# wendongbi/Bridged-GNN

Hardware: AMD Instinct MI355X
Metric: aggregated_edges_per_sec_ktgnn_fwd (higher is better)
Workload: dtype f32; 1 GPU; C4 synthetic bridged graph (local) N=1000000 E'=20991058, 2-layer KT-GNN eval fwd F=128 hidden=128 C=2; parallelism=single, execution=eager launches

## Files before the change

### bridged_gnn_amd/_lib.py

```python
import ctypes as C
import os

import torch

_HERE = os.path.dirname(os.path.abspath(__file__))
SO_PATH = os.path.join(_HERE, "csrc", "libbgnn_hip.so")
_lib = None

_P, _I64, _I32, _F32, _SZ, _INT = C.c_void_p, C.c_int64, C.c_int32, C.c_float, C.c_size_t, C.c_int

SIGNATURES = {
    "bgnn_version": (_INT, []),
    "bgnn_source_hash": (C.c_char_p, []),
    "bgnn_error_string": (C.c_char_p, [_INT]),
    "bgnn_csr_workspace_bytes": (_SZ, [_I64, _I64]),
    "bgnn_build_dst_csr": (_INT, [_P, _I64, _I64, _INT, _P, _P, _P, _P, _P, _SZ, _P]),
    "bgnn_domain_sums_f64": (_INT, [_P, _I64, _I32, _I64, _P, _P, _P]),
    "bgnn_domain_sums_workspace_bytes": (_SZ, [_I32]),
    "bgnn_domain_sums_ws_f64": (_INT, [_P, _I64, _I32, _I64, _P, _P, _P, _SZ, _P]),
    "bgnn_domain_delta_f32": (_INT, [_P, _I32, _P, _P]),
    "bgnn_adaptedconv_transform_f32": (_INT, [_P, _I64, _I32, _I64, _P, _P, _P, _I32, _I32, _P, _P, _P, _P,
                                               _P, _P, _P, _P, _I64, _I64, _I64, _I64, _P, _P, _I32, _P, _P]),
    "bgnn_classifier_stage_f32": (_INT, [_P, _I64, _I32, _I64, _P, _P, _I32, _I32, _P, _P, _P, _P, _P, _P, _P, _P, _I64, _I64,
                                          _P, _P, _I32, _INT, _P, _P, _P, _P, _P, _P]),
    "bgnn_linear_narrow_transform_f32": (_INT, [_P, _I64, _I32, _I64, _P, _P, _I32, _INT, _P, _P, _P, _P, _P, _P]),
    "bgnn_narrow_transform_finish_f32": (_INT, [_P, _I64, _P, _P, _I32, _P, _P, _P, _P, _P, _P, _I64, _P, _P]),
    "bgnn_gram_workspace_bytes": (C.c_size_t, [_I32, _I32]),
    "bgnn_gram_f32": (_INT, [_P, _I64, _I32, _P, _I64, _I32, _I64, _P, _P, C.c_size_t, _P]),
    "bgnn_transform_bwd_prep_workspace_bytes": (C.c_size_t, [_I64, _I32]),
    "bgnn_transform_bwd_prep_f32": (_INT, [_P, _I64, _I64, _I32, _P, _P, _I64, _I32, _P, _P, _P, _P, _P, _P, _I32, _I64, _P, _I64, _P, _P, C.c_size_t, _P]),
    "bgnn_bn_acc_doubles": (_I64, [_I32]),
    "bgnn_bn_relu_dropout_f32": (_INT, [_P, _I64, _I32, _I64, _P, _P, _F32, _INT, _F32, C.c_uint64, _P, _F32, _P, _P, _P, _I64, _P, _P]),
    "bgnn_bn_relu_dropout_bwd_f32": (_INT, [_P, _P, _I64, _I32, _I64, _I64, _P, _P, _P, _F32, _INT, _F32, C.c_uint64, _P, _P, _I64, _P, _P]),
    "bgnn_bn_colstats_f32": (_INT, [_P, _I64, _I32, _I64, _P, _P]),
    "bgnn_bn_apply_rows_f32": (_INT, [_P, _I64, _I32, _I64, _P, _I64, _P, _P, _F32, _INT, _F32, C.c_uint64, _P, _P, _I64, _F32, _P, _P, _P, _I64, _P]),
    "bgnn_bn_bwd_reduce_rows_f32": (_INT, [_P, _P, _I64, _I32, _I64, _I64, _P, _I64, _P, _P, _F32, _INT, _F32, C.c_uint64, _P, _P, _I64, _P, _P]),
    "bgnn_bn_bwd_apply_rows_f32": (_INT, [_P, _P, _I64, _I32, _I64, _I64, _P, _P, _I64, _P, _P, _F32, _INT, _F32, C.c_uint64, _P, _P, _I64, _P, _I64, _P]),
    "bgnn_transform_bwd_consts_f32": (_INT, [_P, _P, _P, _P, _P, _I32, _I32, _P, _P, _P, _P]),
    "bgnn_transform_bwd_finish_f32": (_INT, [_P, _P, _P, _P, _P, _P, _P, _I32, _I32, _I32, _P, _P, _P, _P, _P, _P, _P, _I64, _P]),
    "bgnn_rowdot_f32": (_INT, [_P, _I64, _I64, _I32, _P, _I64, _I32, _P, _P]),
    "bgnn_linear_f32": (_INT, [_P, _I64, _I32, _I64, _P, _P, _I32, _INT, _P, _P, _P, _I64, _P]),
    "bgnn_adaptedconv_aggregate_f32": (_INT, [_P, _P, _I64, _P, _P, _P, _P, _P, _I64, _I64, _I32, _F32,
                                               _P, _I64, _P, _P, _P, _INT, _P, _INT, _I64, _I32, _P, _P, _P]),
    "bgnn_adaptedconv_aggregate_bounded_f32": (_INT, [_P, _P, _I64, _P, _P, _P, _P, _P, _I64, _I64, _I32, _F32,
                                                       _P, _I64, _P, _P, _P, _INT, _P, _INT, _I64, _I32, _P, _P, _I64, _I32, _P]),
    "bgnn_aggregate_tile_queue_words": (_I64, []),
    "bgnn_adaptedconv_aggregate_queued_f32": (_INT, [_P, _P, _I64, _P, _P, _P, _P, _P, _I64, _I64, _I32, _F32,
                                                      _P, _I64, _P, _P, _P, _INT, _P, _INT, _I64, _I32, _P, _P, _I64, _I64, _I32, _P]),
    "bgnn_aggregate_hub_workspace_bytes": (C.c_size_t, [_I64, _I32, _I64]),
    "bgnn_adaptedconv_aggregate_hub_f32": (_INT, [_P, _P, _I64, _P, _P, _P, _P, _P, _I64, _I32, _F32, _P, _I64, _P, _P, _INT, _P, _I32, _P,
                                                   _P, _I32, _P, _I64, _P, _P, _P, _I64, _P, _P, C.c_size_t, _P]),
    "bgnn_adaptedconv_aggregate_bwd_f32": (_INT, [_P, _P, _I64, _P, _P, _P, _P, _P, _I64, _I64, _I32, _F32,
                                                   _P, _I64, _P, _P, _I64, _P, _P, _P, _P, _P]),
    "bgnn_aggregate_bwd_pull_workspace_bytes": (C.c_size_t, [_I64, _I64, _I64, _I32, _I64, _I64]),
    "bgnn_adaptedconv_aggregate_bwd_pull_f32": (_INT, [_P, _P, _I64, _P, _P, _P, _P, _P, _P, _P, _P, _I64, _I64, _I32, _F32,
                                                        _P, _I64, _P, _P, _I64, _P, _P, _P, _P, _I32,
                                                        _P, _I64, _P, _P, _P, _I64, _P, _I64, _P, _P, _P, _I64, _P, C.c_size_t, _P]),
    "bgnn_aggregate_heads_bwd_workspace_bytes": (C.c_size_t, [_I64, _I64, _I32, _I64, _I64]),
    "bgnn_adaptedconv_aggregate_heads_bwd_f32": (_INT, [_P, _P, _P, _P, _P, _P, _P, _P, _P, _I64, _I64, _I32, _I32, _F32,
                                                         _P, _P, _P, _INT, _P, _P, _P, _P, _I32,
                                                         _P, _I64, _P, _P, _P, _I64, _P, _I64, _P, _P, _P, _I64, _P, C.c_size_t, _P]),
    "bgnn_adaptedconv_aggregate_heads_wide_f32": (_INT, [_P, _P, _I64, _P, _P, _P, _P, _P, _I64, _I32, _I32, _F32, _P, _P, _P]),
    "bgnn_aggregate_heads_wide_bwd_workspace_bytes": (C.c_size_t, [_I64, _I32, _I64]),
    "bgnn_adaptedconv_aggregate_heads_wide_bwd_f32": (_INT, [_P, _P, _I64, _P, _P, _P, _P, _P, _P, _P, _I64, _I32, _I32, _F32,
                                                              _P, _P, _P, _P, _P, _P, _P, _P, C.c_size_t, _P]),
    "bgnn_l2_normalize_rows_f32": (_INT, [_P, _I64, _I32, _F32, _P, _P]),
    "bgnn_topk_workspace_bytes": (_SZ, [_I64, _I64, _I32]),
    "bgnn_cosine_topk_f32": (_INT, [_P, _P, _I64, _I64, _I32, _I32, _INT, _P, _P, _P, _P, _SZ, _P]),
    "bgnn_mlp_pair_topk_f32": (_INT, [_P, _P, _P, _P, _P, _F32, _I64, _I64, _I32, _I32, _INT, _P, _P, _P,
                                       _P, _SZ, _P]),
    "bgnn_topk_edges_i64": (_INT, [_P, _I64, _I32, _I64, _I64, _P, _P]),
    "bgnn_topk_edges_coalesced_workspace_bytes": (_SZ, [_I64, _I32]),
    "bgnn_topk_edges_coalesced_i64": (_INT, [_P, _I64, _I32, _I64, _I64, _I64, _P, _P, _SZ, _P]),
    "bgnn_gather_rows_f32": (_INT, [_P, _I64, _I64, _P, _I64, _I32, _P, _I64, _P]),
    "bgnn_coalesce_workspace_bytes": (_SZ, [_I64]),
    "bgnn_coalesce_i64": (_INT, [_P, _I64, _I64, _P, _P, _SZ, _P]),
    "bgnn_sage_mean_aggregate_f32": (_INT, [_P, _I64, _I64, _P, _I64, _P, _P, _I64, _I32, _INT, _INT, _F32, C.c_uint64, _P,
                                             _P, _P, _I64, _P]),
    "bgnn_rows_segment_add_f32": (_INT, [_P, _I64, _I64, _P, _P, _P, _I64, _I32, _INT, _P, _I64, _I64, _P]),
    "bgnn_pair_mlp_workspace_bytes": (_SZ, [_I64]),
    "bgnn_pair_mlp_stats_f32": (_INT, [_P, _I64, _I64, _P, _I64, _I64, _P, _P, _I64, _F32, _P, _P, _P, _P, _SZ, _P]),
    "bgnn_pair_mlp_loss_f32": (_INT, [_P, _I64, _I64, _P, _I64, _I64, _P, _P, _P, _I64, _P, _P, _P, _P, _P, _F32, _P, _P, _P, _P,
                                       _SZ, _P]),
    "bgnn_pair_mlp_segsum_f32": (_INT, [_P, _I64, _I64, _P, _I64, _I64, _P, _P, _P, _I64, _P, _P, _P, _P, _P, _P, _F32, _P, _I64, _P]),
    "bgnn_pair_mlp_eval_f32": (_INT, [_P, _I64, _I64, _P, _I64, _I64, _P, _P, _P, _I64, _P, _P, _P, _P, _P, _P, _P, _SZ, _P]),
    "bgnn_pair_mlp_count_workspace_bytes": (_SZ, [_I64, _I64]),
    "bgnn_pair_mlp_count_f32": (_INT, [_P, _I64, _I64, _P, _I64, _I64, _P, _I64, _P, _I64, _P, _P, _P, _P, _P, _P, _P, _P, _SZ, _P]),
    "bgnn_pair_cos_loss_workspace_bytes": (_SZ, [_I64]),
    "bgnn_pair_cos_count_workspace_bytes": (_SZ, [_I64, _I64]),
    "bgnn_pair_cos_loss_f32": (_INT, [_P, _I64, _I64, _P, _I64, _I64, _P, _P, _P, _I64, _P, _P, _P, _P, _SZ, _P]),
    "bgnn_pair_cos_segsum_f32": (_INT, [_P, _I64, _I64, _P, _P, _P, _I64, _P, _I64, _P, _I64, _P]),
    "bgnn_pair_cos_count_f32": (_INT, [_P, _I64, _I64, _P, _I64, _I64, _P, _I64, _P, _I64, _P, _P, _P, _P, _SZ, _P]),
    "bgnn_sage_mean_aggregate_bwd_workspace_bytes": (_SZ, [_I64, _I32]),
    "bgnn_sage_mean_aggregate_bwd_f32": (_INT, [_P, _I64, _P, _I64, _P, _I64, _P, _P, _I64, _I32, _INT, _F32, _P, _I64, _P, _I64,
                                                 _P, _SZ, _P]),
    "bgnn_gcn_aggregate_workspace_bytes": (_SZ, [_I64, _I32]),
    "bgnn_gcn_aggregate_f32": (_INT, [_P, _I64, _I64, _P, _P, _P, _P, _I64, _I64, _I32, _INT, _F32, C.c_uint64, _P,
                                       _I32, _P, _I64, _P, _P, _I64, _P, _SZ, _P, _P, _I64, _P]),
    "bgnn_gcn_aggregate_bwd_f32": (_INT, [_P, _I64, _P, _I64, _I64, _P, _P, _P, _I64, _I64, _I32, _INT, _F32,
                                           _I32, _P, _I64, _P, _P, _I64, _P, _SZ, _P, _I64, _P, _I64, _P]),
    "bgnn_appnp_propagate_workspace_bytes": (_SZ, [_I64, _I32, _I64]),
    "bgnn_appnp_propagate_f32": (_INT, [_P, _I64, _P, _P, _P, _I64, _I64, _I32, _I32, _F32, _INT,
                                         _I32, _P, _I64, _P, _P, _I64, _P, _SZ, _P, _I64, _P]),
    "bgnn_appnp_log_softmax_bwd_f32": (_INT, [_P, _I64, _P, _I64, _I64, _I32, _P, _I64, _P]),
    "bgnn_feature_dropout_f32": (_INT, [_P, _P, _I64, _I32, _INT, _F32, C.c_uint64, _P, _P, _P]),
    "bgnn_feature_dropout_bwd_f32": (_INT, [_P, _P, _I64, _I32, _INT, _F32, C.c_uint64, _P, _P, _P]),
    "bgnn_appnp_step_f32": (_INT, [_P, _I64, _I64, _P, _I64, _P, _P, _P, _I64, _I64, _I32, _F32, _INT, _INT,
                                    _I32, _P, _I64, _P, _P, _I64, _P, _SZ, _P, _I64, _P]),
    "bgnn_feature_dropout_rows_f32": (_INT, [_P, _P, _P, _I64, _I32, _INT, _F32, C.c_uint64, _P, _P, _P]),
# ... 153 lines not shown
```

### bridged_gnn_amd/classifier_stage.py

```python
import os

import torch
import torch.nn.functional as F

from . import ops
from .ktgnn import _AggregateFn, _AggregateHeadsFn, _AggregateWideHeadsFn, _TransformPairFn, _pad_cols4, _plist


class ClassifierStage:

    def __init__(self, model):
        base = model.clf_base
        self.model, self.convs = model, (base, model.clf_target, model.clf_target)
        self.C, self.ld, self.slope = base.out_channels, ops.pad4(base.out_channels), base.negative_slope
        self.plain = not (base.root_weight or base.normalize)
        self.fused_log_softmax = ops.heads_log_softmax_supported(3, self.C)
        self.drop_caches()

    def drop_caches(self):
        self._a3_key = self._tf_key = self._tf_pack = None

    def views(self, t2s, s2t):
        ld = self.ld
        return [(t2s[:, j * ld:(j + 1) * ld], s2t[:, j * ld:(j + 1) * ld]) for j in range(3)]

    def attention(self, autograd=False):
        if autograd:
            return (torch.stack([c.a_f_t2s.weight.reshape(-1) for c in self.convs]),
                    torch.stack([c.a_f_s2t.weight.reshape(-1) for c in self.convs]))
        key = (self.convs[0]._versions(), self.convs[1]._versions())
        if self._a3_key != key:
            self._a3 = (torch.stack([c.a_f_t2s.weight.detach().reshape(-1) for c in self.convs]).contiguous(),
                        torch.stack([c.a_f_s2t.weight.detach().reshape(-1) for c in self.convs]).contiguous())
            self._a3_key = key
        return self._a3

    def finish(self, out3):
        logp = out3.view(out3.shape[0], 3, self.ld)[:, :, :self.C]
        if not self.fused_log_softmax:
            logp = F.log_softmax(logp, dim=2)
        return logp[:, 0], logp[:, 1], logp[:, 2]

    def fold_transformer(self):
        l0, bn, _, l3 = self.model.clf_transformer
        key = tuple((p.data_ptr(), p._version) for p in _plist(self.model.clf_transformer)) + \
            (bn.running_mean._version, bn.running_var._version)
        if self._tf_key != key:
            s = (bn.weight / torch.sqrt(bn.running_var + bn.eps)).detach()
            self._tf_w0 = (l0.weight.detach() * s[:, None]).float().contiguous()
            self._tf_w0t = self._tf_w0.t().contiguous()
            self._tf_b0 = (l0.bias.detach() * s + bn.bias.detach() - bn.running_mean * s).float().contiguous()
            self._tf_key = key
            self._tf_pack = None

    def transformer_hidden_eval(self, x, mask_u8=None, want_sums=False, sums_out=None):
        self.fold_transformer()
        sums = None
        dout, din = self._tf_w0.shape
        if x.dtype == torch.float32 and x.stride(1) == 1 and ops.linear_supported(din, dout):
            if want_sums:
                sums = sums_out if sums_out is not None else torch.zeros(2 * dout + 2, dtype=torch.float64, device=x.device)
            h1 = ops.linear(x, self._tf_w0, self._tf_b0, relu=True, mask_u8=mask_u8 if want_sums else None, colsum=sums)
        elif hasattr(torch, "_addmm_activation"):
            h1 = torch._addmm_activation(self._tf_b0, x, self._tf_w0t, use_gelu=False)
        else:
            h1 = F.relu(torch.addmm(self._tf_b0, x, self._tf_w0t))
        return (h1, sums) if want_sums else h1

    def transformer_eval(self, x):
        l3 = self.model.clf_transformer[3]
        return F.linear(self.transformer_hidden_eval(x), l3.weight, l3.bias)

    def composed_target_pack(self, din_pad):
        c, l3 = self.convs[1], self.model.clf_transformer[3]
        key = (din_pad, c._versions(), l3.weight._version, l3.bias._version, l3.weight.data_ptr())
        if self._tf_pack is None or self._tf_pack[0] != key:
            W3, b3 = l3.weight.detach(), l3.bias.detach()
            hd = c.head()
            din = W3.shape[0]

            def comp_gate(g):
                g = g.reshape(-1)
                return torch.cat((W3.t() @ g[:din], W3.t() @ g[din:])), (b3 * g[:din]).sum()
            g1, c1 = comp_gate(hd["g_s2t"])
            g2, c2 = comp_gate(hd["g_t2s"])
            head = {"W_s": hd["W_s"] @ W3, "W_t": hd["W_t"] @ W3,
                    "b_s": hd["W_s"] @ b3 + (hd["b_s"] if hd["b_s"] is not None else 0),
                    "b_t": hd["W_t"] @ b3 + (hd["b_t"] if hd["b_t"] is not None else 0),
                    "g_s2t": g1, "g_t2s": g2, "gate_const": (c1, c2)}
            self._tf_pack = (key, ops.pack_transform_heads([head], din_pad))
        return self._tf_pack[1]

    def one_pass(self, x, mask_u8, sums_h, views, arena):
        if sums_h is None or x.dtype != torch.float32 or x.stride(1) != 1:
            return None
        self.fold_transformer()
        dout, din = self._tf_w0.shape
        if x.shape[1] != din or dout != 128:
            return None
        pack_t = self.composed_target_pack(ops.pad4(dout))
        pair = self.convs[0].packed(x.shape[1], self.convs[1])
        if not ops.classifier_stage_supported(x, pair, self._tf_w0, pack_t):
            return None
        n_s = 2 * ops.pad4(dout) + 2
        sums_t = arena.take(n_s) if arena is not None else torch.zeros(n_s, dtype=torch.float64, device=x.device)
        raw = ops.classifier_stage(x, mask_u8, sums_h, pair, [views[0], views[1]], self._tf_w0, self._tf_b0, sums_t, pack_t, relu=True)
        return raw, None, sums_t

    def pair_tables(self, x, mask_u8, sums_h, views):
        self.convs[0].transform(x, mask_u8, sums=sums_h, partner=self.convs[1], out=[views[0], views[1]])

    def target_stage_a(self, x, mask_u8, sums_out=None):
        self.fold_transformer()
        dout, din = self._tf_w0.shape
        pack = self.composed_target_pack(ops.pad4(dout))
        if (sums_out is not None and x.dtype == torch.float32 and x.stride(1) == 1 and x.shape[1] == din
                and ops.linear_narrow_supported(din, dout, pack) and os.environ.get("BGNN_FUSED_TARGET", "1") != "0"):
            return ops.linear_narrow_transform(x, self._tf_w0, self._tf_b0, mask_u8, sums_out, pack, relu=True), None, sums_out
        h1, sums1 = self.transformer_hidden_eval(x, mask_u8, want_sums=True, sums_out=sums_out)
        h1 = _pad_cols4(h1)
        if sums1 is None or sums1.numel() != 2 * h1.shape[1] + 2:
            sums1 = ops.domain_sums(h1, mask_u8)
        return None, h1, sums1

    def target_stage_b(self, stage_a, mask_u8, out, sums_t=None):
        raw, h1, sums_t = (*stage_a[:2], sums_t if sums_t is not None else stage_a[2])
        if raw is not None:
            ops.narrow_transform_finish(raw, mask_u8, sums_t, self.composed_target_pack(ops.pad4(self._tf_w0.shape[0])), out)
        else:
            ops.adaptedconv_transform(h1, mask_u8, None, self.composed_target_pack(h1.shape[1]), out=[out], sums=sums_t)

    def target_tables(self, x, mask_u8, out, arena=None, sums_out=None):
        if sums_out is None:
            n_s = 2 * ops.pad4(self.model.clf_transformer[0].weight.shape[0]) + 2
            sums_out = arena.take(n_s) if arena is not None else torch.zeros(n_s, dtype=torch.float64, device=x.device)
        self.target_stage_b(self.target_stage_a(x, mask_u8, sums_out), mask_u8, out)

    def eval_tables(self, x, mask_u8, sums_h, views, arena):
        a = self.one_pass(x, mask_u8, sums_h, views, arena)
        if a is not None:
            return self.target_stage_b(a, mask_u8, views[2])
        self.pair_tables(x, mask_u8, sums_h, views)
        self.target_tables(x, mask_u8, views[2], arena)

    def train_walk(self, opt_in=False):
        if ops.heads_log_softmax_supported(3, self.C) and not (opt_in and os.environ.get("BGNN_FUSED_TRAIN_HEADS", "1") == "0"):
            return "narrow"
        if ops.wide_heads_supported(3, self.C) and not (opt_in and os.environ.get("BGNN_WIDE_TRAIN_HEADS", "0") != "1"):
            return "wide"
        return None if opt_in else "convs"

    def train_tables(self, x, mask_u8, sums_x, bn, sums_of=None, mean_hook=None):
        base, target, _ = self.convs
        l0, bnm, _, l3 = self.model.clf_transformer
        xt = l3(bn(l0(x), bnm, True, 0.0)).contiguous()
        sums_t = sums_of(xt) if sums_of is not None else None
        if mean_hook is None and _TransformPairFn.supported(x, base, target):
            prm = [t for c in (base, target)
                   for t in (c.lin_s.weight, c.lin_s.bias, c.lin_t.weight, c.lin_t.bias, c.a_g_s2t.weight, c.a_g_t2s.weight)]
            tabs_x = _TransformPairFn.apply(x, mask_u8, base, target, sums_x, *prm)
        else:
            tabs_x = (*base._transform_autograd(x, mask_u8, sums_x, mean_hook), *target._transform_autograd(x, mask_u8, sums_x, mean_hook))
        return (*tabs_x, *target._transform_autograd(xt, mask_u8, sums_t, mean_hook))

    def train_aggregate(self, walk, csr, mask_u8, tables, n_rows=None):
        C = self.C
        a_t, a_s = self.attention(autograd=True)
        if walk == "convs":
            return tuple(F.log_softmax(_AggregateFn.apply(tables[2 * j], tables[2 * j + 1], a_t[j], a_s[j], csr, mask_u8, C,
                                                          c.negative_slope)[:n_rows, :C], dim=1) for j, c in enumerate(self.convs))
        fn = _AggregateHeadsFn if walk == "narrow" else _AggregateWideHeadsFn
        logp = fn.apply(csr, mask_u8, C, self.slope, a_t, a_s, *tables)[:n_rows, :, :C]
        return logp[:, 0], logp[:, 1], logp[:, 2]
```

### bridged_gnn_amd/csrc/bgnn_aggregate.hip

```cpp
#include <cstdlib>
#include <cstring>
#include <type_traits>
#include "bgnn_common.h"

namespace {

struct AggParams {
  const float* h_t2s;
  const float* h_s2t;
  int64_t ldh;
  const float* a_t2s;
  const float* a_s2t;
  const int32_t* rowptr;
  const int32_t* col;
  const uint8_t* mask;
  int64_t row_begin;
  int64_t row_end;
  int32_t D;
  float slope;
  float* out;
  int64_t ldo;
  float* alpha;
  const float* ep_scale;
  const float* ep_shift;
// ... 1050 lines not shown
        __builtin_amdgcn_sched_barrier(0);
#pragma unroll
        for (int u = 0; u < U; ++u) asm volatile("buffer_load_dwordx4 %0, %1, %2, 0 offen" : "=v"(v[u]) : "v"(off[u]), "s"(rt) : "memory");
        xoff += (uint32_t)(STEP * 4);
        u32x4_t nq;
        request(nq);
        if constexpr (SLOW) asm volatile("s_waitcnt vmcnt(4)" : "+v"(v[0]), "+v"(v[1]), "+v"(v[2]), "+v"(v[3]) : : "memory");
        else asm volatile("s_waitcnt vmcnt(1)" : "+v"(v[0]), "+v"(v[1]), "+v"(v[2]), "+v"(v[3]) : : "memory");
        __builtin_amdgcn_sched_barrier(0);
        float l[U], cm = -INFINITY;
#pragma unroll
        for (int u = 0; u < U; ++u) {
          f2 z0 = f2{v[u].x, v[u].y} + h01, z1 = f2{v[u].z, v[u].w} + h23;
          z0 = __builtin_elementwise_max(z0, z0 * sl);
          z1 = __builtin_elementwise_max(z1, z1 * sl);
          float t = a4.x * z0.x;
          t = fmaf(a4.y, z0.y, t);
          t = fmaf(a4.z, z1.x, t);
          t = fmaf(a4.w, z1.y, t);
          l[u] = rem > u * EP ? t : -INFINITY;
          cm = fmaxf(cm, l[u]);
        }
        const float mn = fmaxf(m, cm);
        const float sc = (m == mn) ? 1.f : __expf(m - mn);
        const f2 sc2 = {sc, sc};
        acc01 *= sc2; acc23 *= sc2;
#pragma unroll
        for (int u = 0; u < U; ++u) {
          const float pe = (l[u] == -INFINITY) ? 0.f : __expf(l[u] - mn);
          s = u == 0 ? fmaf(s, sc, pe) : s + pe;
          acc01.x = fmaf(pe, v[u].x, acc01.x); acc01.y = fmaf(pe, v[u].y, acc01.y);
          acc23.x = fmaf(pe, v[u].z, acc23.x); acc23.y = fmaf(pe, v[u].w, acc23.y);
        }
        m = mn;
        rem -= STEP;
        uint32_t nid[U];
        take(nq, nid);
        offsets(nid);
      }
    };
    if (any) {
      if (slow) walk(std::true_type{});
      else walk(std::false_type{});
    }
    float4 acc = make_float4(acc01.x, acc01.y, acc23.x, acc23.y);
#pragma unroll
    for (int o = 1; o < EP; o <<= 1) {
      const int src = (sub ^ o) * HEADS + h + g * GL;
      const int from = lane_on ? src : lane;
      const float m2 = __shfl(m, from), s2 = __shfl(s, from);
      float4 b;
      b.x = __shfl(acc.x, from); b.y = __shfl(acc.y, from); b.z = __shfl(acc.z, from); b.w = __shfl(acc.w, from);
      const float mn = fmaxf(m, m2);
      const float c1 = (m == mn) ? 1.f : __expf(m - mn), c2 = (m2 == mn) ? 1.f : __expf(m2 - mn);
      s = fmaf(s, c1, s2 * c2);
      acc.x = fmaf(acc.x, c1, b.x * c2); acc.y = fmaf(acc.y, c1, b.y * c2);
      acc.z = fmaf(acc.z, c1, b.z * c2); acc.w = fmaf(acc.w, c1, b.w * c2);
      m = mn;
    }
    if (rvalid && sub == 0) {
#pragma clang fp contract(off)
      const float inv = 1.f / (s + 1e-16f);
      float4 r4 =make_float4(acc.x * inv, acc.y * inv, acc.z * inv, acc.w * inv);
      if (p.ep_relu == 2) {
        float mx = r4.x;
        if (p.D > 1) mx = fmaxf(mx, r4.y);
        if (p.D > 2) mx = fmaxf(mx, r4.z);
        if (p.D > 3) mx = fmaxf(mx, r4.w);
        float se = expf(r4.x - mx);
        if (p.D > 1) se += expf(r4.y - mx);
        if (p.D > 2) se += expf(r4.z - mx);
        if (p.D > 3) se += expf(r4.w - mx);
        const float lse = logf(se);
        r4.x = r4.x - mx - lse;
        r4.y = p.D > 1 ? r4.y - mx - lse : 0.f;
        r4.z = p.D > 2 ? r4.z - mx - lse : 0.f;
        r4.w = p.D > 3 ? r4.w - mx - lse : 0.f;
      }
      __builtin_amdgcn_raw_buffer_store_b128(__builtin_bit_cast(u32x4_t, r4), ro, ((uint32_t)i * (uint32_t)HEADS + (uint32_t)h) * 16u, 0, 0);
    }
  }
}

inline int tq_chunk_for(int64_t ntiles, int64_t grid) {
  static const int forced = [] { const char* e = getenv("BGNN_AGG_CHUNK"); return e ? atoi(e) : 0; }();
  (void)ntiles; (void)grid;
  return forced > 0 ? forced : 4;
}

template <int HEADS, int EP, int U>
int launch_heads(const AggParams& p, hipStream_t st) {
  constexpr int RPB = 4 * (64 / (EP * HEADS));
  static const int cap = [] {
    int per_cu = 0, dev = 0;
    hipDeviceProp_t prop;
    if (hipGetDevice(&dev) != hipSuccess || hipGetDeviceProperties(&prop, dev) != hipSuccess) return 2048;
    if (hipOccupancyMaxActiveBlocksPerMultiprocessor(&per_cu, agg_heads_lanes_kernel<HEADS, EP, U>, 256, 0) != hipSuccess || per_cu < 1) return 2048;
    if (per_cu > 8) per_cu = 8;
    return per_cu * prop.multiProcessorCount / 8 * 8;
  }();
  const int64_t ntiles = (p.row_end - p.row_begin + p.n_vrows + RPB - 1) / RPB;
  int64_t grid = ntiles < cap ? (ntiles + 7) / 8 * 8 : cap;
  if (grid < 8) grid = 8;
  hipLaunchKernelGGL((agg_heads_lanes_kernel<HEADS, EP, U>), dim3((unsigned)grid), dim3(256), 0, st, p);
  BGNN_LAUNCH_CHECK();
  return 0;
}

template <int LF, int EP, int U>
int resident_blocks() {
  static const int nb = [] {
    int per_cu = 0, dev = 0;
    hipDeviceProp_t prop;
    if (hipGetDevice(&dev) != hipSuccess || hipGetDeviceProperties(&prop, dev) != hipSuccess) return 2048;
    if (hipOccupancyMaxActiveBlocksPerMultiprocessor(&per_cu, agg_kernel<LF, EP, U>, 256, 0) != hipSuccess || per_cu < 1)
      return 2048;
    if (per_cu > 8) per_cu = 8;
    return per_cu * prop.multiProcessorCount / 8 * 8;
  }();
  return nb;
}

template <int LF, int EP, int U>
int launch(const AggParams& p, hipStream_t st) {
  constexpr int RPB = 4 * (64 / (LF * EP));
  int64_t ntiles = ((p.row_end - p.row_begin) * p.heads + RPB - 1) / RPB;
  const int64_t cap = resident_blocks<LF, EP, U>();
  int64_t grid = ntiles < cap ? (ntiles + 7) / 8 * 8 : cap;
  if (grid < 8) grid = 8;
  AggParams q = p;
  q.tq_chunk = tq_chunk_for(ntiles, grid);
  hipLaunchKernelGGL((agg_kernel<LF, EP, U>), dim3((unsigned)grid), dim3(256), 0, st, q);
  BGNN_LAUNCH_CHECK();
  return 0;
}

template <int LF, int U>
int launch_wide(const AggParams& p, hipStream_t st) {
  constexpr int RPB = 4 * (64 / LF);
  static const int cap = [] {
    int per_cu = 0, dev = 0;
    hipDeviceProp_t prop;
    if (hipGetDevice(&dev) != hipSuccess || hipGetDeviceProperties(&prop, dev) != hipSuccess) return 2048;
    if (hipOccupancyMaxActiveBlocksPerMultiprocessor(&per_cu, agg_wide_kernel<LF, U>, 256, 0) != hipSuccess || per_cu < 1) return 2048;
    if (per_cu > 8) per_cu = 8;
    const char* e = getenv("BGNN_AGG_BLOCKS_PER_CU");
    if (e && atoi(e) > 0 && atoi(e) < per_cu) per_cu = atoi(e);
    return per_cu * prop.multiProcessorCount / 8 * 8;
  }();
  const int64_t ntiles = ((p.row_end - p.row_begin) * p.heads + p.n_vrows + RPB - 1) / RPB;
  int64_t grid = ntiles < cap ? (ntiles + 7) / 8 * 8 : cap;
  if (grid < 8) grid = 8;
  AggParams q = p;
  q.tq_chunk = tq_chunk_for(ntiles, grid);
  static const int il = [] { const char* e = getenv("BGNN_AGG_INTERLEAVE"); return e ? atoi(e) : 1; }();
  q.tq_interleave = il;
  static const int nseg = [] { const char* e = getenv("BGNN_XCD_SEGMENTS"); return e ? atoi(e) : 8; }();
  q.xcd_segments = nseg;
  hipLaunchKernelGGL((agg_wide_kernel<LF, U>), dim3((unsigned)grid), dim3(256), 0, st, q);
  BGNN_LAUNCH_CHECK();
  return 0;
}

static bool fast_plan(AggParams& p, int64_t table_rows) {
  static const bool on = [] { const char* e = getenv("BGNN_AGG_FAST"); return !(e && atoi(e) == 0); }();
  if (!on || table_rows <= 0) return false;
  if (p.heads != 1 || p.mode != 0 || p.n_vrows != 0 || p.hub_threshold != 0) return false;
  const int64_t lim24 = (int64_t)1 << 24, lim32 = ((int64_t)1 << 32) - 1;
  if (table_rows > lim24 || p.row_end > table_rows || p.ldh * 4 >= lim24 || p.ldo * 4 >= lim24) return false;
  const char* a = reinterpret_cast<const char*>(p.h_t2s);
  const char* b = reinterpret_cast<const char*>(p.h_s2t);
  const char* lo = a < b ? a : b;
  const int64_t span = (int64_t)((a < b ? b : a) - lo) + table_rows * p.ldh * 4;
  if (span > lim32 || p.row_end * p.ldo * 4 > lim32) return false;
  p.tbl_base = lo;
  p.tbl_bytes = (uint32_t)span;
  p.off_t2s = (uint32_t)(a - lo);
  p.off_s2t = (uint32_t)(b - lo);
  const int64_t lane_max = (span - table_rows * p.ldh * 4) + p.ldh * 4, dead = (((int64_t)1 << 32) - 16) - lane_max;
  p.dead_off = dead >= span ? (uint32_t)dead : 0u;
  return true;
}

static bool heads_fast_plan(AggParams& p, int64_t table_rows) {
  static const bool on = [] { const char* e = getenv("BGNN_HEADS_FAST"); return !(e && atoi(e) == 0); }();
  if (!on || table_rows <= 0) return false;
  if ((p.heads != 2 && p.heads != 3) || p.D > 4 || p.ldh != 4 || p.ldo != 4) return false;
  if (p.mode != 0 || p.n_vrows != 0 || p.hub_threshold != 0 || p.alpha != nullptr) return false;
  if (!(p.slope >= 0.f && p.slope <= 1.f)) return false;
  const int64_t lim24 = (int64_t)1 << 24, lim32 = ((int64_t)1 << 32) - 1;
  const int64_t rs = (int64_t)p.heads * 16;
  if (table_rows > lim24 || p.row_end > table_rows) return false;
  const char* a = reinterpret_cast<const char*>(p.h_t2s);
  const char* b = reinterpret_cast<const char*>(p.h_s2t);
  const char* lo = a < b ? a : b;
  const int64_t span = (int64_t)((a < b ? b : a) - lo) + table_rows * rs;
  if (span > lim32 || p.row_end * rs > lim32) return false;
  p.tbl_base = lo;
  p.tbl_bytes = (uint32_t)span;
  p.off_t2s = (uint32_t)(a - lo);
  p.off_s2t = (uint32_t)(b - lo);
  p.dead_off = (uint32_t)span;
  return true;
}

constexpr int kClaimTileDefault = 1;
struct ClaimCfg { int tile, nq, ahead; };
static const ClaimCfg& claim_cfg() {
  static const ClaimCfg c = [] {
    ClaimCfg r{kClaimTileDefault, 4, 1};
    if (const char* e = getenv("BGNN_AGG_CLAIM")) r.tile = strcmp(e, "chunk") == 0 ? 0 : (strcmp(e, "tile") == 0 ? 1 : r.tile);
    if (const char* e = getenv("BGNN_AGG_SUBQUEUES")) { const int v = atoi(e); if (v >= 1 && v <= 8) r.nq = v; }
    if (const char* e = getenv("BGNN_AGG_CLAIM_AHEAD")) r.ahead = atoi(e) != 0;
    return r;
  }();
  return c;
}
static int64_t claim_queue_words() { return (int64_t)8 * claim_cfg().nq * TQ_SPACING_WORDS; }

template <int LF, bool ALPHA>
int launch_wide_fast(const AggParams& p, hipStream_t st) {
  constexpr int RPB = 4 * (64 / LF);
  static const int per_cu_max = [] {
    int per_cu = 0;
    if (hipOccupancyMaxActiveBlocksPerMultiprocessor(&per_cu, agg_wide_fast_kernel<LF, ALPHA>, 256, 0) != hipSuccess || per_cu < 1) return 0;
    if (per_cu > 8) per_cu = 8;
    const char* e = getenv("BGNN_AGG_BLOCKS_PER_CU");
    if (e && atoi(e) > 0 && atoi(e) < per_cu) per_cu = atoi(e);
    return per_cu;
  }();
  static const int n_cu = [] {
    int dev = 0;
    hipDeviceProp_t prop;
    if (hipGetDevice(&dev) != hipSuccess || hipGetDeviceProperties(&prop, dev) != hipSuccess) return 0;
    return prop.multiProcessorCount;
  }();
  static const bool forced = getenv("BGNN_AGG_BLOCKS_PER_CU") != nullptr;
  int per_cu = per_cu_max;
  if (p.gather_hint == 2 && !forced && per_cu > 3) per_cu = 3;
  const int64_t cap = (per_cu_max > 0 && n_cu > 0) ? (int64_t)per_cu * n_cu / 8 * 8 : 2048;
  const int64_t ntiles = (p.row_end - p.row_begin + RPB - 1) / RPB;
  int64_t grid = ntiles < cap ? (ntiles + 7) / 8 * 8 : cap;
  if (grid < 8) grid = 8;
  AggParams q = p;
  q.tq_chunk = tq_chunk_for(ntiles, grid);
  static const int il = [] { const char* e = getenv("BGNN_AGG_INTERLEAVE"); return e ? atoi(e) : 1; }();
  q.tq_interleave = il;
  static const int nseg = [] { const char* e = getenv("BGNN_XCD_SEGMENTS"); return e ? atoi(e) : 8; }();
  q.xcd_segments = nseg;
  const ClaimCfg& cc = claim_cfg();
  const bool tile_claims = cc.tile && p.tile_queue != nullptr && p.tq_words >= claim_queue_words();
  q.tq_subqueues = tile_claims ? cc.nq : 0;
  q.tq_ahead = cc.ahead;
  hipLaunchKernelGGL((agg_wide_fast_kernel<LF, ALPHA>), dim3((unsigned)grid), dim3(256), 0, st, q);
  BGNN_LAUNCH_CHECK();
  return 0;
}

struct HubMergeParams {
  const int32_t* hub_rows; const int32_t* seg_ptr; int64_t n_hubs;
  const float* part_acc;
  const float* part_ms;
  const uint8_t* mask;
  int32_t D; int64_t ldo; int32_t heads;
  float* out; const float* ep_scale; const float* ep_shift; int ep_relu;
  double* colsum; float* state_ms;
  float* alpha; const int32_t* rowptr;
};

template <int LF>
__global__ __launch_bounds__(256) void hub_merge_wide_kernel(HubMergeParams p) {
  const int lane = threadIdx.x % LF, grp = threadIdx.x / LF;
  constexpr int GPB = 256 / LF;
  const int f0 = lane * 4;
// ... 52 lines not shown
      *reinterpret_cast<float4*>(p.out + node * p.ldo + f0) = o;
      if (p.mask[node] != 0) { cs_s.x += o.x; cs_s.y += o.y; cs_s.z += o.z; cs_s.w += o.w; n_s += 1.f; }
      else                   { cs_t.x += o.x; cs_t.y += o.y; cs_t.z += o.z; cs_t.w += o.w; n_t += 1.f; }
    }
  }
  if (p.colsum != nullptr) {
    unsafeAtomicAdd(&red[0][f0], cs_s.x); unsafeAtomicAdd(&red[0][f0 + 1], cs_s.y);
    unsafeAtomicAdd(&red[0][f0 + 2], cs_s.z); unsafeAtomicAdd(&red[0][f0 + 3], cs_s.w);
    unsafeAtomicAdd(&red[1][f0], cs_t.x); unsafeAtomicAdd(&red[1][f0 + 1], cs_t.y);
    unsafeAtomicAdd(&red[1][f0 + 2], cs_t.z); unsafeAtomicAdd(&red[1][f0 + 3], cs_t.w);
    if (lane == 0) { unsafeAtomicAdd(&red[0][LF * 4], n_s); unsafeAtomicAdd(&red[1][LF * 4], n_t); }
    __syncthreads();
    for (int t = threadIdx.x; t < 2 * (LF * 4 + 1); t += 256) {
      const int d = t / (LF * 4 + 1), c = t % (LF * 4 + 1);
      const double sum = (double)red[d][c];
      if (c == LF * 4) unsafeAtomicAdd(&p.colsum[2 * p.ldo + d], sum);
      else if (c < p.ldo) unsafeAtomicAdd(&p.colsum[d * p.ldo + c], sum);
    }
  }
}

__global__ __launch_bounds__(256) void hub_merge_heads_kernel(HubMergeParams p) {
  const int64_t t = (int64_t)blockIdx.x * 256 + threadIdx.x;
  if (t >= p.n_hubs * p.heads) return;
  const int64_t hrow = t / p.heads;
  const int h = (int)(t - hrow * p.heads);
  const int64_t node = p.hub_rows[hrow];
  float m = -INFINITY, s = 0.f;
  float4 acc = make_float4(0.f, 0.f, 0.f, 0.f);
  for (int32_t v = p.seg_ptr[hrow]; v < p.seg_ptr[hrow + 1]; ++v) {
    const int64_t e = (int64_t)v * p.heads + h;
    const float m2 = p.part_ms[2 * e], s2 = p.part_ms[2 * e + 1];
    const float4 b = *reinterpret_cast<const float4*>(p.part_acc + e * p.ldo);
    const float mn = fmaxf(m, m2);
    const float c1 = (m == mn) ? 1.f : __expf(m - mn), c2 = (m2 == mn) ? 1.f : __expf(m2 - mn);
    s = s * c1 + s2 * c2;
    acc.x = acc.x * c1 + b.x * c2; acc.y = acc.y * c1 + b.y * c2;
    acc.z = acc.z * c1 + b.z * c2; acc.w = acc.w * c1 + b.w * c2;
    m = mn;
  }
  const float inv = 1.f / (s + 1e-16f);
  float4 r = make_float4(acc.x * inv, acc.y * inv, acc.z * inv, acc.w * inv);
  if (p.state_ms != nullptr) {
    p.state_ms[2 * (node * p.heads + h)] = m;
    p.state_ms[2 * (node * p.heads + h) + 1] = s;
  }
  if (p.ep_relu == 2) {
    float mx = r.x;
    if (p.D > 1) mx = fmaxf(mx, r.y);
    if (p.D > 2) mx = fmaxf(mx, r.z);
    if (p.D > 3) mx = fmaxf(mx, r.w);
    float se = expf(r.x - mx);
    if (p.D > 1) se += expf(r.y - mx);
    if (p.D > 2) se += expf(r.z - mx);
    if (p.D > 3) se += expf(r.w - mx);
    const float lse = logf(se);
    r.x = r.x - mx - lse;
    r.y = p.D > 1 ? r.y - mx - lse : 0.f;
    r.z = p.D > 2 ? r.z - mx - lse : 0.f;
    r.w = p.D > 3 ? r.w - mx - lse : 0.f;
  }
  *reinterpret_cast<float4*>(p.out + (node * p.heads + h) * p.ldo) = r;
}

template <int HEADS, int EP, int U>
int launch_heads_fast(const AggParams& p, hipStream_t st) {
  constexpr int RPB = 4 * (64 / (EP * HEADS));
  static const int cap = [] {
    int per_cu = 0, dev = 0;
    hipDeviceProp_t prop;
    if (hipGetDevice(&dev) != hipSuccess || hipGetDeviceProperties(&prop, dev) != hipSuccess) return 2048;
    if (hipOccupancyMaxActiveBlocksPerMultiprocessor(&per_cu, agg_heads_fast_kernel<HEADS, EP, U>, 256, 0) != hipSuccess || per_cu < 1) return 2048;
    if (per_cu > 8) per_cu = 8;
    return per_cu * prop.multiProcessorCount / 8 * 8;
  }();
  const int64_t ntiles = (p.row_end - p.row_begin + RPB - 1) / RPB;
  int64_t grid = ntiles < cap ? (ntiles + 7) / 8 * 8 : cap;
  if (grid < 8) grid = 8;
  hipLaunchKernelGGL((agg_heads_fast_kernel<HEADS, EP, U>), dim3((unsigned)grid), dim3(256), 0, st, p);
  BGNN_LAUNCH_CHECK();
  return 0;
}

static int dispatch_aggregate(const AggParams& p, hipStream_t st, int64_t table_rows = 0) {
  const int32_t D = p.D, heads = p.heads;
  if ((heads == 3 || heads == 2) && D <= 4 && p.ldh == 4 && p.ldo == 4) {
    AggParams q = p;
    if (heads_fast_plan(q, table_rows)) return heads == 3 ? launch_heads_fast<3, 2, 4>(q, st) : launch_heads_fast<2, 2, 4>(q, st);
    return heads == 3 ? launch_heads<3, 2, 4>(p, st) : launch_heads<2, 2, 4>(p, st);
  }
  const int nv = (D + 3) / 4;
  if (nv <= 1) return launch<1, 4, 4>(p, st);
  if (nv <= 2) return launch<2, 2, 4>(p, st);
  if (nv <= 4) return launch<4, 1, 8>(p, st);
  if (nv <= 8) return launch<8, 1, 4>(p, st);
  const bool wide_ok = p.slope >= 0.f && p.slope <= 1.f && (int64_t)heads * p.ldh * 4 < (int64_t)1 << 32;
  if (wide_ok) {
    AggParams q = p;
    if (fast_plan(q, table_rows)) {
      if (q.alpha != nullptr) {
        if (nv <= 16) return launch_wide_fast<16, true>(q, st);
        if (nv <= 32) return launch_wide_fast<32, true>(q, st);
        return launch_wide_fast<64, true>(q, st);
      }
      if (nv <= 16) return launch_wide_fast<16, false>(q, st);
      if (nv <= 32) return launch_wide_fast<32, false>(q, st);
      return launch_wide_fast<64, false>(q, st);
    }
    if (nv <= 16) return launch_wide<16, 4>(p, st);
    if (nv <= 32) return launch_wide<32, 4>(p, st);
    return launch_wide<64, 4>(p, st);
  }
  if (nv <= 16) return launch<16, 1, 8>(p, st);
  if (nv <= 32) return launch<32, 1, 4>(p, st);
  return launch<64, 1, 4>(p, st);
}

static bool hub_capable(int32_t D, int64_t ldh, int64_t ldo, int32_t heads, float slope) {
  if ((heads == 3 || heads == 2) && D <= 4 && ldh == 4 && ldo == 4) return true;
  const int nv = (D + 3) / 4;
  return heads == 1 && nv > 8 && slope >= 0.f && slope <= 1.f && ldh * 4 < (int64_t)1 << 32;
}

}

static int aggregate_impl(const float* h_t2s, const float* h_s2t, int64_t ldh,
                          const float* a_t2s, const float* a_s2t,
                          const int32_t* rowptr, const int32_t* col, const uint8_t* mask,
                          int64_t row_begin, int64_t row_end, int32_t D, float negative_slope,
                          float* out, int64_t ldo, float* alpha_opt,
                          const float* ep_scale_opt, const float* ep_shift_opt, int ep_relu,
                          float* state_ms_opt, int part, int64_t park_begin, int32_t heads,
                          double* colsum_opt, uint32_t* tile_queue_opt, int64_t tile_queue_words, int64_t table_rows, int32_t gather_hint,
                          void* stream) {
  if (colsum_opt && heads != 1) return BGNN_E_SHAPE;
  if (tile_queue_opt && tile_queue_words < 8) return BGNN_E_WORKSPACE;
  if (part == 1 && (park_begin < row_begin || park_begin > row_end)) return BGNN_E_SHAPE;
  if (part < 0 || part > 3 || (part != 0 && (!state_ms_opt || alpha_opt))) return BGNN_E_NULL;
  if (part == 3 && !((heads == 3 || heads == 2) && D <= 4 && ldh == 4 && ldo == 4)) return BGNN_E_SHAPE;
  if (heads < 1 || heads > 8 || (heads > 1 && (alpha_opt || ep_scale_opt))) return BGNN_E_SHAPE;
  if (ep_relu < 0 || ep_relu > 2) return BGNN_E_SHAPE;
  if (ep_relu == 2 && !((heads == 3 || heads == 2) && D <= 4 && ldh == 4 && ldo == 4)) return BGNN_E_SHAPE;
  if (!h_t2s || !h_s2t || !a_t2s || !a_s2t || !rowptr || !col || !mask || !out) return BGNN_E_NULL;
  if (row_begin < 0 || row_end < row_begin || D <= 0 || D > 256 || ldh < D || ldo < D) return BGNN_E_SHAPE;
  if ((ldh & 3) || (ldo & 3) || !bgnn_aligned16(h_t2s) || !bgnn_aligned16(h_s2t) || !bgnn_aligned16(out))
    return BGNN_E_ALIGN;
  if ((ep_scale_opt == nullptr) != (ep_shift_opt == nullptr)) return BGNN_E_NULL;
  if (row_end == row_begin) return 0;
  AggParams p{h_t2s, h_s2t, ldh, a_t2s, a_s2t, rowptr, col, mask, row_begin, row_end, D, negative_slope,
              out, ldo, alpha_opt, ep_scale_opt, ep_shift_opt, ep_relu, tile_queue_opt, colsum_opt, heads, state_ms_opt, part,
              park_begin, 4};
  p.gather_hint = gather_hint;
  p.tq_words = tile_queue_words;
  hipStream_t st = (hipStream_t)stream;
  if (tile_queue_opt) {
    const int64_t zw = claim_cfg().tile && tile_queue_words >= claim_queue_words() ? claim_queue_words() : 8;
    hipError_t e = bgnn_zero_async(tile_queue_opt, (size_t)zw * sizeof(uint32_t), st);
    if (e != hipSuccess) return (int)e;
  }
  return dispatch_aggregate(p, st, table_rows);
}

extern "C" int bgnn_adaptedconv_aggregate_f32(const float* h_t2s, const float* h_s2t, int64_t ldh,
                                              const float* a_t2s, const float* a_s2t,
                                              const int32_t* rowptr, const int32_t* col, const uint8_t* mask,
                                              int64_t row_begin, int64_t row_end, int32_t D, float negative_slope,
                                              float* out, int64_t ldo, float* alpha_opt,
                                              const float* ep_scale_opt, const float* ep_shift_opt, int ep_relu,
                                              float* state_ms_opt, int part, int64_t park_begin, int32_t heads,
                                              double* colsum_opt, uint32_t* tile_queue_opt, void* stream) {
  return aggregate_impl(h_t2s, h_s2t, ldh, a_t2s, a_s2t, rowptr, col, mask, row_begin, row_end, D, negative_slope, out, ldo, alpha_opt,
                        ep_scale_opt, ep_shift_opt, ep_relu, state_ms_opt, part, park_begin, heads, colsum_opt, tile_queue_opt, 8, 0, 0, stream);
}

extern "C" int bgnn_adaptedconv_aggregate_bounded_f32(const float* h_t2s, const float* h_s2t, int64_t ldh,
                                                      const float* a_t2s, const float* a_s2t,
                                                      const int32_t* rowptr, const int32_t* col, const uint8_t* mask,
                                                      int64_t row_begin, int64_t row_end, int32_t D, float negative_slope,
                                                      float* out, int64_t ldo, float* alpha_opt,
                                                      const float* ep_scale_opt, const float* ep_shift_opt, int ep_relu,
                                                      float* state_ms_opt, int part, int64_t park_begin, int32_t heads,
                                                      double* colsum_opt, uint32_t* tile_queue_opt, int64_t table_rows, int32_t gather_hint,
                                                      void* stream) {
  if (table_rows < row_end || gather_hint < 0 || gather_hint > 2) return BGNN_E_SHAPE;
  return aggregate_impl(h_t2s, h_s2t, ldh, a_t2s, a_s2t, rowptr, col, mask, row_begin, row_end, D, negative_slope, out, ldo, alpha_opt,
                        ep_scale_opt, ep_shift_opt, ep_relu, state_ms_opt, part, park_begin, heads, colsum_opt, tile_queue_opt, 8, table_rows, gather_hint, stream);
}

extern "C" int64_t bgnn_aggregate_tile_queue_words(void) { return claim_cfg().tile ? claim_queue_words() : 8; }

extern "C" int bgnn_adaptedconv_aggregate_queued_f32(const float* h_t2s, const float* h_s2t, int64_t ldh,
                                                     const float* a_t2s, const float* a_s2t,
                                                     const int32_t* rowptr, const int32_t* col, const uint8_t* mask,
                                                     int64_t row_begin, int64_t row_end, int32_t D, float negative_slope,
                                                     float* out, int64_t ldo, float* alpha_opt,
                                                     const float* ep_scale_opt, const float* ep_shift_opt, int ep_relu,
                                                     float* state_ms_opt, int part, int64_t park_begin, int32_t heads,
                                                     double* colsum_opt, uint32_t* tile_queue_opt, int64_t tile_queue_words,
                                                     int64_t table_rows, int32_t gather_hint, void* stream) {
  if (table_rows < row_end || gather_hint < 0 || gather_hint > 2) return BGNN_E_SHAPE;
  return aggregate_impl(h_t2s, h_s2t, ldh, a_t2s, a_s2t, rowptr, col, mask, row_begin, row_end, D, negative_slope, out, ldo, alpha_opt,
                        ep_scale_opt, ep_shift_opt, ep_relu, state_ms_opt, part, park_begin, heads, colsum_opt, tile_queue_opt,
                        tile_queue_words, table_rows, gather_hint, stream);
}

extern "C" size_t bgnn_aggregate_hub_workspace_bytes(int64_t n_segments, int32_t heads, int64_t ldo) {
  const size_t nv = (size_t)(n_segments > 0 ? n_segments : 0), h = (size_t)(heads > 0 ? heads : 1);
  return bgnn_align_up(sizeof(float) * nv * h * (size_t)(ldo > 0 ? ldo : 0), 256) + bgnn_align_up(sizeof(float) * 2 * nv * h, 256) + 256;
}

extern "C" int bgnn_adaptedconv_aggregate_hub_f32(const float* h_t2s, const float* h_s2t, int64_t ldh,
                                                  const float* a_t2s, const float* a_s2t,
                                                  const int32_t* rowptr, const int32_t* col, const uint8_t* mask,
                                                  int64_t N, int32_t D, float negative_slope, float* out, int64_t ldo,
                                                  const float* ep_scale_opt, const float* ep_shift_opt, int ep_relu,
                                                  float* state_ms_opt, int32_t heads, double* colsum_opt,
                                                  uint32_t* tile_queue_opt, int32_t hub_threshold, const int32_t* hub_rows,
                                                  int64_t n_hubs, const int32_t* hub_seg_ptr, const int32_t* seg_bounds,
                                                  const int32_t* seg_node, int64_t n_segments, float* alpha_opt,
                                                  void* ws, size_t ws_bytes, void* stream) {
  if (!h_t2s || !h_s2t || !a_t2s || !a_s2t || !rowptr || !col || !mask || !out) return BGNN_E_NULL;
  if (alpha_opt && heads != 1) return BGNN_E_SHAPE;
  if (n_hubs > 0 && (!hub_rows || !hub_seg_ptr || !seg_bounds || !seg_node || !ws)) return BGNN_E_NULL;
  if (N < 0 || D <= 0 || D > 256 || ldh < D || ldo < D || (ldh & 3) || (ldo & 3) || hub_threshold < 2 || n_hubs < 0 || n_segments < n_hubs)
    return BGNN_E_SHAPE;
  if (!hub_capable(D, ldh, ldo, heads, negative_slope)) return BGNN_E_SHAPE;
  if (colsum_opt && heads != 1) return BGNN_E_SHAPE;
  if (heads > 1 && ep_scale_opt) return BGNN_E_SHAPE;
  if (ep_relu < 0 || ep_relu > 2 || (ep_relu == 2 && heads == 1)) return BGNN_E_SHAPE;
  if ((ep_scale_opt == nullptr) != (ep_shift_opt == nullptr)) return BGNN_E_NULL;
  if (!bgnn_aligned16(h_t2s) || !bgnn_aligned16(h_s2t) || !bgnn_aligned16(out) || (ws && !bgnn_aligned16(ws))) return BGNN_E_ALIGN;
  if (n_hubs > 0 && ws_bytes < bgnn_aggregate_hub_workspace_bytes(n_segments, heads, ldo)) return BGNN_E_WORKSPACE;
  if (N == 0) return 0;
  hipStream_t st = (hipStream_t)stream;
  const int part = (state_ms_opt && heads > 1) ? 3 : 0;
  AggParams p{h_t2s, h_s2t, ldh, a_t2s, a_s2t, rowptr, col, mask, 0, N, D, negative_slope,
              out, ldo, alpha_opt, ep_scale_opt, ep_shift_opt, ep_relu, tile_queue_opt, colsum_opt, heads, state_ms_opt, part,
              0, 4};
  p.hub_threshold = n_hubs > 0 ? hub_threshold : 0;
  if (tile_queue_opt) {
    hipError_t e = bgnn_zero_async(tile_queue_opt, 8 * sizeof(uint32_t), st);
    if (e != hipSuccess) return (int)e;
  }
  float* part_acc = n_hubs > 0 ? (float*)ws : nullptr;
  float* part_ms = n_hubs > 0 ? (float*)((char*)ws + bgnn_align_up(sizeof(float) * (size_t)n_segments * (size_t)heads * (size_t)ldo, 256)) : nullptr;
  if (n_hubs > 0) {
    p.vrow_node = seg_node; p.vrow_bounds = seg_bounds; p.n_vrows = n_segments; p.vout = part_acc; p.vms = part_ms;
  }
  int rc = dispatch_aggregate(p, st, N);
  if (rc || n_hubs == 0) return rc;
  HubMergeParams mp{hub_rows, hub_seg_ptr, n_hubs, part_acc, part_ms, mask, D, ldo, heads, out, ep_scale_opt, ep_shift_opt,
                    ep_relu, colsum_opt, part == 3 ? state_ms_opt : nullptr, alpha_opt, rowptr};
  if (heads > 1) {
    hipLaunchKernelGGL(hub_merge_heads_kernel, dim3((unsigned)((n_hubs * heads + 255) / 256)), dim3(256), 0, st, mp);
  } else {
    const int nvs = (D + 3) / 4;
    int64_t grid = n_hubs < 2048 ? n_hubs : 2048;
    if (nvs <= 16) hipLaunchKernelGGL(hub_merge_wide_kernel<16>, dim3((unsigned)((grid + 15) / 16)), dim3(256), 0, st, mp);
    else if (nvs <= 32) hipLaunchKernelGGL(hub_merge_wide_kernel<32>, dim3((unsigned)((grid + 7) / 8)), dim3(256), 0, st, mp);
    else hipLaunchKernelGGL(hub_merge_wide_kernel<64>, dim3((unsigned)((grid + 3) / 4)), dim3(256), 0, st, mp);
  }
  BGNN_LAUNCH_CHECK();
  return 0;
}

#ifdef BGNN_TUNING
extern "C" int bgnn_tune_reset_counters(void* stream) { (void)stream; return 0; }
extern "C" int bgnn_tune_aggregate(const float* h_t2s, const float* h_s2t, int64_t ldh, const float* a_t2s,
                                   const float* a_s2t, const int32_t* rowptr, const int32_t* col, const uint8_t* mask,
// ... 41 lines not shown
```

### bridged_gnn_amd/csrc/bgnn_transform.hip

```cpp
#include <cstdlib>
#include <type_traits>
#include "bgnn_common.h"
#include "bgnn_transform_params.h"

using bgnn_tf::GemmParams;
using bgnn_tf::MAXH;
using bgnn_tf::f32x16;
using bgnn_tf::tanh_fast;

namespace {

constexpr int DS_NT = 1024;
__global__ __launch_bounds__(DS_NT) void domain_sums_kernel(const float* __restrict__ x, int64_t N, int32_t Din,
                                                          int64_t ldx, const uint8_t* __restrict__ mask,
                                                          double* __restrict__ sums, double* __restrict__ part) {
  if (part != nullptr) sums = part + (int64_t)blockIdx.x * (2 * Din + 2);
  const int nc4 = Din >> 2;
  const int cw = nc4 < 256 ? nc4 : 256;
  const int rl = DS_NT / cw;
  const int tid = threadIdx.x;
  const int cl = tid % cw, r0 = tid / cw;
  const bool active = r0 < rl;
  const int64_t rows_per_block = (N + gridDim.x - 1) / gridDim.x;
  const int64_t rb = blockIdx.x * rows_per_block;
// ... 834 lines not shown
                                              const uint8_t* mask, const float* delta_opt, const double* sums_opt,
                                              int32_t n_heads, int32_t D, const float* Wp, const float* bias_p,
                                              const float* gates, const float* gate_const_opt,
                                              float* h_s2t_0, float* h_t2s_0, float* h_s2t_1, float* h_t2s_1,
                                              int64_t ldh, int64_t row_stride, int64_t n_tail_t2s, int64_t n_tail_s2t,
                                              const int32_t* tile_need_opt, const int64_t* team_runs_host_opt, int32_t n_team_runs,
                                              float* small_ws, void* stream) {
  if ((delta_opt != nullptr) == (sums_opt != nullptr)) return BGNN_E_NULL;
  if (delta_opt && !bgnn_aligned16(delta_opt)) return BGNN_E_ALIGN;
  if (n_team_runs < 0 || n_team_runs > 2 || (n_team_runs > 0 && !team_runs_host_opt)) return BGNN_E_SHAPE;
  if (tile_need_opt && (n_tail_t2s || n_tail_s2t)) return BGNN_E_SHAPE;
  if (n_tail_t2s < 0 || n_tail_s2t < 0 || n_tail_t2s + n_tail_s2t > N) return BGNN_E_SHAPE;
  if (!x || !mask || !Wp || !bias_p || !gates || !h_s2t_0 || !h_t2s_0 || !small_ws) return BGNN_E_NULL;
  if (n_heads < 1 || n_heads > MAXH || (n_heads == 2 && (!h_s2t_1 || !h_t2s_1))) return BGNN_E_NULL;
  if (N < 0 || Din <= 0 || D <= 0 || ldx < Din || ldh < D) return BGNN_E_SHAPE;
  if ((Din & 3) || (ldx & 3) || (ldh & 3) || (row_stride & 3) || row_stride < ldh) return BGNN_E_SHAPE;
  if (!bgnn_aligned16(x) || !bgnn_aligned16(Wp) || !bgnn_aligned16(gates)) return BGNN_E_ALIGN;
  if (N == 0) return 0;
  hipStream_t st = (hipStream_t)stream;
  const int NC = n_heads * 2 * (int)ldh;
  float* wd = small_ws;
  float* gc = small_ws + NC;
  hipLaunchKernelGGL(wd_kernel, dim3((unsigned)((NC + 2 * n_heads + 3) / 4)), dim3(256), 0, st, Wp, NC, Din, delta_opt, sums_opt, gates,
                     gate_const_opt, n_heads, wd, gc);
  BGNN_LAUNCH_CHECK();
  GemmParams p{};
  p.x = x; p.ldx = ldx; p.N = N; p.Din = Din; p.mask = mask; p.Wp = Wp; p.bias = bias_p; p.wd = wd; p.g = gates; p.gc = gc;
  p.out[0][0] = h_s2t_0; p.out[0][1] = h_t2s_0; p.out[1][0] = h_s2t_1; p.out[1][1] = h_t2s_1;
  p.ldh = ldh; p.row_stride = row_stride; p.NC = NC; p.n_heads = n_heads; p.relu = 0; p.colsum = nullptr; p.col_off = 0;
  const int64_t nrt = (N + BM - 1) / BM;
  const int64_t nrt8 = (nrt + 7) / 8 * 8;
  const bool wreg = NC % 64 == 0 && Din <= 128;
  p.tail_t2s_begin = 0; p.tail_s2t_begin = 0;
  if ((n_tail_t2s || n_tail_s2t) && n_heads == 1 && wreg) {
    p.tail_t2s_begin = N - n_tail_t2s - n_tail_s2t;
    p.tail_s2t_begin = N - n_tail_s2t;
    if (p.tail_s2t_begin == 0) p.tail_s2t_begin = 1, p.tail_t2s_begin = p.tail_t2s_begin > 1 ? 1 : p.tail_t2s_begin;
  }
  static const bool use_stream = [] { const char* e = getenv("BGNN_GEMM_STREAM"); return !e || atoi(e) != 0; }();
  p.tile_need = tile_need_opt;
  for (int r = 0; r < n_team_runs; ++r) {
    p.team_begin[r] = team_runs_host_opt[3 * r]; p.team_end[r] = team_runs_host_opt[3 * r + 1]; p.team_table[r] = (int32_t)team_runs_host_opt[3 * r + 2];
  }
  if (use_stream && bgnn_tf_stream_supported(p)) return bgnn_tf_stream_launch(p, st, n_cu());
  if (wreg) return launch_wreg<0>(p, st);
  if (NC <= 24 && Din <= 128) {
    const int64_t nt = (N + 31) / 32, nb = (nt + 3) / 4;
    const unsigned grid = (unsigned)(nb < 2 * n_cu() ? nb : 2 * n_cu());
    if (Din <= 64) hipLaunchKernelGGL((transform_skinny_kernel<64>), dim3(grid), dim3(256), 0, st, p);
    else hipLaunchKernelGGL((transform_skinny_kernel<128>), dim3(grid), dim3(256), 0, st, p);
  } else if (NC <= 32) {
    hipLaunchKernelGGL((transform_gemm_kernel<32, 4, 1, 1, 1>), dim3((unsigned)nrt8), dim3(256), 0, st, p);
  } else if (NC <= 64) {
    hipLaunchKernelGGL((transform_gemm_kernel<64, 2, 2, 2, 1>), dim3((unsigned)nrt8), dim3(256), 0, st, p);
  } else {
    const int nct = (NC + 127) / 128;
    hipLaunchKernelGGL((transform_gemm_kernel<128, 2, 2, 2, 2>), dim3((unsigned)(nrt8 * nct)), dim3(256), 0, st, p);
  }
  BGNN_LAUNCH_CHECK();
  return 0;
}

extern "C" int bgnn_linear_f32(const float* x, int64_t N, int32_t Din, int64_t ldx, const float* W, const float* bias,
                               int32_t Dout, int relu, const uint8_t* mask_opt, double* colsum_opt,
                               float* out, int64_t ldo, void* stream) {
  if (!x || !W || !bias || !out || (colsum_opt && !mask_opt)) return BGNN_E_NULL;
  if (N < 0 || Din <= 0 || Din > 128 || (Din & 3) || (ldx & 3) || ldx < Din || Dout <= 0 || (Dout & 63) || ldo < Dout || (ldo & 3))
    return BGNN_E_SHAPE;
  if (!bgnn_aligned16(x) || !bgnn_aligned16(W) || !bgnn_aligned16(bias) || !bgnn_aligned16(out)) return BGNN_E_ALIGN;
  if (N == 0) return 0;
  GemmParams p{};
  p.x = x; p.ldx = ldx; p.N = N; p.Din = Din; p.mask = mask_opt; p.Wp = W; p.bias = bias; p.wd = nullptr; p.g = nullptr; p.gc = nullptr;
  p.out[0][0] = out; p.out[0][1] = out; p.out[1][0] = out; p.out[1][1] = out;
  p.ldh = Dout;
  p.row_stride = ldo; p.NC = Dout; p.n_heads = 1; p.relu = relu; p.colsum = colsum_opt;
  return launch_wreg<1>(p, (hipStream_t)stream);
}

namespace {
__global__ __launch_bounds__(256) void narrow_finish_kernel(const float* __restrict__ raw, int64_t N,
                                                            const uint8_t* __restrict__ mask,
                                                            const float* __restrict__ bias, const float* __restrict__ wd,
                                                            const float* __restrict__ gc, float* __restrict__ out_s2t,
                                                            float* __restrict__ out_t2s, int64_t row_stride) {
  const float4 b0 = *reinterpret_cast<const float4*>(bias), b1 = *reinterpret_cast<const float4*>(bias + 4);
  const float4 w0 = *reinterpret_cast<const float4*>(wd), w1 = *reinterpret_cast<const float4*>(wd + 4);
  const float g0 = gc[0], g1 = gc[1];
  for (int64_t r = blockIdx.x * (int64_t)blockDim.x + threadIdx.x; r < N; r += (int64_t)gridDim.x * blockDim.x) {
    const float4 a = *reinterpret_cast<const float4*>(raw + r * 12);
    const float4 b = *reinterpret_cast<const float4*>(raw + r * 12 + 4);
    const float2 pg = *reinterpret_cast<const float2*>(raw + r * 12 + 8);
    const bool sdom = mask[r] != 0;
    const float c0 = sdom ? -tanh_fast(pg.x + g0) : 0.f;
    const float c1 = sdom ? 0.f : tanh_fast(pg.y + g1);
    float4 o0, o1;
    o0.x = fmaf(c0, w0.x, a.x + b0.x); o0.y = fmaf(c0, w0.y, a.y + b0.y);
    o0.z = fmaf(c0, w0.z, a.z + b0.z); o0.w = fmaf(c0, w0.w, a.w + b0.w);
    o1.x = fmaf(c1, w1.x, b.x + b1.x); o1.y = fmaf(c1, w1.y, b.y + b1.y);
    o1.z = fmaf(c1, w1.z, b.z + b1.z); o1.w = fmaf(c1, w1.w, b.w + b1.w);
    *reinterpret_cast<float4*>(out_s2t + r * row_stride) = o0;
    *reinterpret_cast<float4*>(out_t2s + r * row_stride) = o1;
  }
}
}

extern "C" int bgnn_linear_narrow_transform_f32(const float* x, int64_t N, int32_t Din, int64_t ldx, const float* W,
                                                const float* bias, int32_t Dout, int relu, const uint8_t* mask,
                                                double* colsum, const float* Wp2, const float* gates2,
                                                float* raw, void* stream) {
  if (!x || !W || !bias || !mask || !colsum || !Wp2 || !gates2 || !raw) return BGNN_E_NULL;
  if (N < 0 || Din <= 0 || Din > 128 || (Din & 3) || (ldx & 3) || ldx < Din || (Dout != 64 && Dout != 128 && Dout != 256))
    return BGNN_E_SHAPE;
  if (!bgnn_aligned16(x) || !bgnn_aligned16(W) || !bgnn_aligned16(bias) || !bgnn_aligned16(raw)) return BGNN_E_ALIGN;
  if (N == 0) return 0;
  GemmParams p{};
  p.x = x; p.ldx = ldx; p.N = N; p.Din = Din; p.mask = mask; p.Wp = W; p.bias = bias;
  p.ldh = Dout; p.row_stride = Dout; p.NC = Dout; p.n_heads = 1; p.relu = relu ? 1 : 0; p.colsum = colsum;
  p.w2 = Wp2; p.g2 = gates2; p.raw = raw;
  return launch_wreg<2>(p, (hipStream_t)stream);
}

extern "C" int bgnn_classifier_stage_f32(const float* x, int64_t N, int32_t Din, int64_t ldx, const uint8_t* mask,
                                         const double* sums_x, int32_t sk_heads, int32_t sk_D, const float* sk_Wp,
                                         const float* sk_bias, const float* sk_gates, const float* sk_gate_const_opt,
                                         float* h_s2t_0, float* h_t2s_0, float* h_s2t_1, float* h_t2s_1, int64_t sk_ldh,
                                         int64_t sk_row_stride, const float* W, const float* bias, int32_t Dout, int relu,
                                         double* colsum, const float* Wp2, const float* gates2, float* raw, float* small_ws,
                                         void* stream) {
  if (!x || !mask || !sums_x || !sk_Wp || !sk_bias || !sk_gates || !h_s2t_0 || !h_t2s_0 || !W || !bias || !colsum || !Wp2 || !gates2 ||
      !raw || !small_ws) return BGNN_E_NULL;
  if (sk_heads < 1 || sk_heads > MAXH || (sk_heads == 2 && (!h_s2t_1 || !h_t2s_1))) return BGNN_E_NULL;
  if (N < 0 || Din <= 0 || (Din & 3) || (ldx & 3) || ldx < Din || sk_D <= 0 || sk_ldh < sk_D || (sk_ldh & 3) || (sk_row_stride & 3) ||
      sk_row_stride < sk_ldh) return BGNN_E_SHAPE;
  if (!bgnn_aligned16(x) || !bgnn_aligned16(sk_Wp) || !bgnn_aligned16(sk_bias) || !bgnn_aligned16(raw) || !bgnn_aligned16(small_ws))
    return BGNN_E_ALIGN;
  if (N == 0) return 0;
  hipStream_t st = (hipStream_t)stream;
  const int sk_NC = sk_heads * 2 * (int)sk_ldh;
  float* wd = small_ws;
  float* gc = small_ws + sk_NC;
  GemmParams p{};
  p.x = x; p.ldx = ldx; p.N = N; p.Din = Din; p.mask = mask; p.Wp = W; p.bias = bias;
  p.ldh = Dout; p.row_stride = Dout; p.NC = Dout; p.n_heads = 1; p.relu = relu ? 1 : 0; p.colsum = colsum;
  p.w2 = Wp2; p.g2 = gates2; p.raw = raw;
  p.sk_Wp = sk_Wp; p.sk_bias = sk_bias; p.sk_wd = wd; p.sk_g = sk_gates; p.sk_gc = gc;
  p.sk_out[0][0] = h_s2t_0; p.sk_out[0][1] = h_t2s_0; p.sk_out[1][0] = h_s2t_1; p.sk_out[1][1] = h_t2s_1;
  p.sk_ldh = sk_ldh; p.sk_row_stride = sk_row_stride; p.sk_NC = sk_NC; p.sk_heads = sk_heads;
  if (!bgnn_tf_cls_supported(p)) return BGNN_E_SHAPE;
  hipLaunchKernelGGL(wd_kernel, dim3((unsigned)((sk_NC + 2 * sk_heads + 3) / 4)), dim3(256), 0, st, sk_Wp, sk_NC, Din, (const float*)nullptr,
                     sums_x, sk_gates, sk_gate_const_opt, sk_heads, wd, gc);
  BGNN_LAUNCH_CHECK();
  return bgnn_tf_cls_launch(p, st, n_cu());
}

extern "C" int bgnn_narrow_transform_finish_f32(const float* raw, int64_t N, const uint8_t* mask, const double* sums,
                                                int32_t Din, const float* Wp2, const float* bias2, const float* gates2,
                                                const float* gate_const_opt, float* h_s2t, float* h_t2s,
                                                int64_t row_stride, float* small_ws, void* stream) {
  if (!raw || !mask || !sums || !Wp2 || !bias2 || !gates2 || !h_s2t || !h_t2s || !small_ws) return BGNN_E_NULL;
  if (N < 0 || Din <= 0 || (Din & 3) || row_stride < 4 || (row_stride & 3)) return BGNN_E_SHAPE;
  if (!bgnn_aligned16(raw) || !bgnn_aligned16(h_s2t) || !bgnn_aligned16(h_t2s) || !bgnn_aligned16(bias2) ||
      !bgnn_aligned16(small_ws)) return BGNN_E_ALIGN;
  if (N == 0) return 0;
  hipStream_t st = (hipStream_t)stream;
  float* wd = small_ws;
  float* gc = small_ws + 8;
  hipLaunchKernelGGL(wd_kernel, dim3(3), dim3(256), 0, st, Wp2, 8, Din, (const float*)nullptr, sums, gates2, gate_const_opt, 1, wd, gc);
  BGNN_LAUNCH_CHECK();
  const int64_t nb = (N + 255) / 256;
  hipLaunchKernelGGL(narrow_finish_kernel, dim3((unsigned)(nb < 4096 ? nb : 4096)), dim3(256), 0, st, raw, N, mask, bias2, wd, gc,
                     h_s2t, h_t2s, row_stride);
  BGNN_LAUNCH_CHECK();
  return 0;
}
```

### bridged_gnn_amd/csrc/bgnn_transform_cls.hip

```cpp
#include <cstdio>
#include <cstdlib>
#include "bgnn_common.h"
#include "bgnn_transform_params.h"

using bgnn_tf::GemmParams;
using bgnn_tf::MAXH;
using bgnn_tf::f32x16;
using bgnn_tf::tanh_fast;

namespace {

typedef _Float16 h8 __attribute__((ext_vector_type(8)));
typedef _Float16 h4 __attribute__((ext_vector_type(4)));

constexpr int CLS_TARGET_EXP = 10;
constexpr int DK = 128, KB16 = DK / 16, NCT = 4;
constexpr int PIECE = 32 * DK * 2;
constexpr int SLOT = 32 * 36 * 4 + 2 * 32 * 4;
constexpr int T_LD = 36;

__device__ __forceinline__ int chunk_off(int r, int c) { return r * 256 + ((c ^ (r & 15)) << 4); }
__device__ __forceinline__ void pow2_scales(float mx, float& sc, float& inv) {
  int E = (__builtin_bit_cast(int, mx) >> 23) & 0xff;
  E = E < 40 ? 40 : E;
// ... 159 lines not shown
  float cs_s[NCT], cs_t[NCT], cnt_s = 0.f, cnt_t = 0.f;
#pragma unroll
  for (int ct = 0; ct < NCT; ++ct) cs_s[ct] = cs_t[ct] = 0.f;

  if (tile < ntiles) gload(tile);
  for (; tile < ntiles; tile += stride) {
    CLS_MARK(0);
    const bool sdom = rmk != 0;
    const int64_t row = tile * 32 + fr;
    const bool valid = row < p.N;
    float mx = 0.f;
#pragma unroll
    for (int kb = 0; kb < KB16; ++kb)
#pragma unroll
      for (int c = 0; c < 2; ++c) {
        if (!din_full && 16 * kb + 8 * fh + 4 * c >= p.Din) ra[kb][c] = make_float4(0.f, 0.f, 0.f, 0.f);
        mx = fmaxf(fmaxf(fabsf(ra[kb][c].x), fabsf(ra[kb][c].y)), mx);
        mx = fmaxf(fmaxf(fabsf(ra[kb][c].z), fabsf(ra[kb][c].w)), mx);
      }
    mx = fmaxf(mx, __shfl_xor(mx, 32));
    float scx, s_row;
    pow2_scales(mx, scx, s_row);
    h8 xh[KB16], xl[KB16];
#pragma unroll
    for (int kb = 0; kb < KB16; ++kb)
#pragma unroll
      for (int c = 0; c < 2; ++c) {
        const float f[4] = {ra[kb][c].x, ra[kb][c].y, ra[kb][c].z, ra[kb][c].w};
#pragma unroll
        for (int e = 0; e < 4; ++e) {
          const _Float16 h = (_Float16)(f[e] * scx);
          xh[kb][4 * c + e] = h;
          xl[kb][4 * c + e] = (_Float16)fmaf(f[e], scx, -(float)h);
        }
      }
    if (fh == 0) {
      cfs[fr] = (valid && sdom) ? 1.f : 0.f;
      cfs[32 + fr] = (valid && !sdom) ? 1.f : 0.f;
      cnt_s += (valid && sdom) ? 1.f : 0.f;
      cnt_t += (valid && !sdom) ? 1.f : 0.f;
    }
    const int64_t tnext = tile + stride < ntiles ? tile + stride : tile;
    if constexpr (!PAIR) gload(tnext);
    __builtin_amdgcn_fence(__ATOMIC_RELEASE, "workgroup", "local");
    constexpr int HK = KB16 / 2;
    h8 wf[2][HK][2];
    auto fetch_w = [&](int hc, int buf) {
      const int op = hc >> 1, half = hc & 1;
      const unsigned char* wb = wl + ((op == 0 ? NCT : op - 1) * 2) * PIECE;
#pragma unroll
      for (int j = 0; j < HK; ++j) {
        wf[buf][j][0] = *reinterpret_cast<const h8*>(wb + roff(HK * half + j));
        wf[buf][j][1] = *reinterpret_cast<const h8*>(wb + PIECE + roff(HK * half + j));
      }
    };
    auto half_chain = [&](int hc, f32x16& acc, auto&& between) {
      if constexpr (PAIR) {
        __builtin_amdgcn_sched_barrier(0);
        fetch_w(hc, 0);
      } else if (hc + 1 < 2 * (NCT + 1)) fetch_w(hc + 1, (hc + 1) & 1);
      __builtin_amdgcn_sched_barrier(0);
      const int half = hc & 1, buf = PAIR ? 0 : hc & 1;
#pragma unroll
      for (int j = 0; j < HK; ++j) {
        const int kb = HK * half + j;
        acc = __builtin_amdgcn_mfma_f32_32x32x16_f16(wf[buf][j][0], xl[kb], acc, 0, 0, 0);
        acc = __builtin_amdgcn_mfma_f32_32x32x16_f16(wf[buf][j][1], xh[kb], acc, 0, 0, 0);
        acc = __builtin_amdgcn_mfma_f32_32x32x16_f16(wf[buf][j][0], xh[kb], acc, 0, 0, 0);
        between(kb);
      }
    };
    auto nothing = [](int) {};
    CLS_MARK(1);
    if constexpr (!PAIR) fetch_w(0, 0);
    {
      f32x16 acc;
#pragma unroll
      for (int r = 0; r < 16; ++r) acc[r] = 0.f;
      half_chain(0, acc, nothing);
      half_chain(1, acc, nothing);
      CLS_MARK(2);
      const float ss = s_row * cinvS;
      if (valid) {
        float cf = 0.f;
#pragma unroll
        for (int q = 0; q < 3; ++q) {
          if (optr[q] != nullptr) {
            if (newq[q]) {
              const float pre = hsel[q] == 0 ? acc[12] : hsel[q] == 1 ? acc[13] : hsel[q] == 2 ? acc[14] : acc[15];
              cf = (sdom != t1q[q]) ? tanh_fast(fmaf(pre, ss, gcq[q])) : 0.f;
              cf = t1q[q] ? cf : -cf;
            }
            const float4 bq = *reinterpret_cast<const float4*>(&skc[0][8 * q + 4 * fh]), wq = *reinterpret_cast<const float4*>(&skc[1][8 * q + 4 * fh]);
            float4 o;
            o.x = fmaf(cf, wq.x, fmaf(acc[4 * q], ss, bq.x));     o.y = fmaf(cf, wq.y, fmaf(acc[4 * q + 1], ss, bq.y));
            o.z = fmaf(cf, wq.z, fmaf(acc[4 * q + 2], ss, bq.z)); o.w = fmaf(cf, wq.w, fmaf(acc[4 * q + 3], ss, bq.w));
            *reinterpret_cast<float4*>(optr[q] + row * p.sk_row_stride) = o;
          }
        }
      }
    }
    float o2[8];
#pragma unroll
    for (int i = 0; i < 8; ++i) o2[i] = 0.f;
    const float sc1 = s_row * cinvW;
    struct Stage2 { float a1[16]; float mx, sc2, inv2; h8 ah[2], al[2]; f32x16 acc2; h8 w2h[2], w2l[2]; };
    auto stage2_step = [&](Stage2& q, int ct, int j) {
      if (j == 0) {
        q.mx = fmaxf(q.mx, __shfl_xor(q.mx, 32));
#pragma unroll
        for (int kb = 0; kb < 2; ++kb) { q.w2h[kb] = w2lds[ct][kb][0][lane]; q.w2l[kb] = w2lds[ct][kb][1][lane]; }
      } else if (j == 1) {
        pow2_scales(q.mx, q.sc2, q.inv2);
#pragma unroll
        for (int r = 0; r < 16; ++r) q.acc2[r] = 0.f;
      } else if (j == 2 || j == 3) {
        const int kb = j - 2;
#pragma unroll
        for (int e = 0; e < 8; ++e) {
          const _Float16 h = (_Float16)(q.a1[8 * kb + e] * q.sc2);
          q.ah[kb][e] = h;
          q.al[kb][e] = (_Float16)fmaf(q.a1[8 * kb + e], q.sc2, -(float)h);
        }
      } else if (j == 4 || j == 5) {
        const int kb = j - 4;
        q.acc2 = __builtin_amdgcn_mfma_f32_32x32x16_f16(q.w2h[kb], q.al[kb], q.acc2, 0, 0, 0);
        q.acc2 = __builtin_amdgcn_mfma_f32_32x32x16_f16(q.w2l[kb], q.ah[kb], q.acc2, 0, 0, 0);
        q.acc2 = __builtin_amdgcn_mfma_f32_32x32x16_f16(q.w2h[kb], q.ah[kb], q.acc2, 0, 0, 0);
      } else if (j == 6) {
#pragma unroll
        for (int r = 0; r < 16; ++r) {
          const float v = tsc[(16 * fh + r) * T_LD + fr];
          cs_s[ct] = fmaf(cfs[16 * fh + r], v, cs_s[ct]);
          cs_t[ct] = fmaf(cfs[32 + 16 * fh + r], v, cs_t[ct]);
        }
        if constexpr (PAIR) asm volatile("" : "+v"(cs_s[ct]), "+v"(cs_t[ct]));
      } else {
        const float s2 = q.inv2 * cinv2;
#pragma unroll
        for (int i = 0; i < 8; ++i) o2[i] = fmaf(q.acc2[i], s2, o2[i]);
        if constexpr (PAIR) asm volatile("" : "+v"(o2[0]), "+v"(o2[1]), "+v"(o2[2]), "+v"(o2[3]), "+v"(o2[4]), "+v"(o2[5]), "+v"(o2[6]), "+v"(o2[7]));
      }
    };
    Stage2 q2;
    f32x16 acc;
#pragma unroll
    for (int r = 0; r < 16; ++r) acc[r] = 0.f;
    CLS_MARK(3);
    half_chain(2, acc, nothing);
    half_chain(3, acc, nothing);
    CLS_MARK(4);
#pragma unroll
    for (int ct = 0; ct < NCT; ++ct) {
      __builtin_amdgcn_fence(__ATOMIC_RELEASE, "workgroup", "local");
      q2.mx = 0.f;
#pragma unroll
      for (int qq = 0; qq < 4; ++qq) {
        const float4 b4 = *reinterpret_cast<const float4*>(&bias1[32 * ct + 8 * qq + 4 * fh]);
        const float bb[4] = {b4.x, b4.y, b4.z, b4.w};
#pragma unroll
        for (int e = 0; e < 4; ++e) {
          float v = fmaf(acc[4 * qq + e], sc1, bb[e]);
          if (relu) v = fmaxf(v, 0.f);
          q2.a1[4 * qq + e] = v;
          q2.mx = fmaxf(q2.mx, fabsf(v));
        }
        *reinterpret_cast<float4*>(&tsc[fr * T_LD + 8 * qq + 4 * fh]) =
            make_float4(q2.a1[4 * qq], q2.a1[4 * qq + 1], q2.a1[4 * qq + 2], q2.a1[4 * qq + 3]);
      }
      CLS_MARK(5);
      if constexpr (PAIR) {
        if (ct + 1 == NCT) gload(tnext);
        __builtin_amdgcn_sched_barrier(0);
#pragma unroll
        for (int j = 0; j < 8; ++j) stage2_step(q2, ct, j);
        __builtin_amdgcn_sched_barrier(0);
        if (ct + 1 < NCT) {
#pragma unroll
          for (int r = 0; r < 16; ++r) acc[r] = 0.f;
          half_chain(2 * (ct + 2), acc, nothing);
// ... 114 lines not shown
```

### bridged_gnn_amd/csrc/bgnn_transform_params.h

```cpp
#pragma once
#include "bgnn_common.h"

namespace bgnn_tf {

typedef float f32x16 __attribute__((ext_vector_type(16)));
constexpr int MAXH = 2;

struct GemmParams {
  const float* x; int64_t ldx; int64_t N; int32_t Din;
  const uint8_t* mask;
  const float* Wp;
  const float* bias;
  const float* wd;
  const float* g;
  const float* gc;
  float* out[MAXH][2];
  int64_t ldh; int64_t row_stride; int32_t NC; int32_t n_heads;
  int32_t relu;
  double* colsum;
  int32_t col_off;
  const float* w2;
  const float* g2;
  float* raw;
  int64_t tail_t2s_begin, tail_s2t_begin;
  const int32_t* tile_need;
  int64_t team_begin[2], team_end[2];
  int32_t team_table[2];
  const float* sk_Wp; const float* sk_bias; const float* sk_wd; const float* sk_g; const float* sk_gc;
  float* sk_out[MAXH][2]; int64_t sk_ldh; int64_t sk_row_stride; int32_t sk_NC; int32_t sk_heads;
};

__device__ __forceinline__ float tanh_fast(float z) { return 1.f - 2.f * __builtin_amdgcn_rcpf(__expf(2.f * z) + 1.f); }

}

int bgnn_tf_stream_launch(const bgnn_tf::GemmParams& p, hipStream_t st, int n_cu);
bool bgnn_tf_stream_supported(const bgnn_tf::GemmParams& p);

int bgnn_tf_cls_launch(const bgnn_tf::GemmParams& p, hipStream_t st, int n_cu);
bool bgnn_tf_cls_supported(const bgnn_tf::GemmParams& p);
```

### bridged_gnn_amd/ktgnn.py

```python
import math
import os
import weakref

import torch
import torch.nn.functional as F
from torch import nn

from . import ops

__all__ = ["Linear", "AdaptedConv", "KTGNN_no_complement"]


def _plist(module):
    pl = module.__dict__.get("_bgnn_plist")
    if pl is None:
        pl = list(module.parameters())
        module.__dict__["_bgnn_plist"] = pl
    return pl


def _forget_plists(root):
    for m in root.modules():
        m.__dict__.pop("_bgnn_plist", None)

# ... 610 lines not shown
    def _prepare(self, data):
        if self.cached_edges and self._csr is not None:
            return self._csr
        csr = ops.build_dst_csr(data.edge_index, data.central_mask.shape[0], rewrite_self_loops=True)
        if self.cached_edges:
            self._csr = csr
        return csr

    def _hidden(self, x, csr, central_mask, want_sums=False, arena=None):
        sums = None
        for ind, conv in enumerate(self.convs):
            sums_in, sums = sums, None
            if self.use_bn and not self.training and not (torch.is_grad_enabled() and any(p.requires_grad for p in _plist(conv))):
                sc, sh = bn_eval_affine(self.bns[ind])
                if arena is None:
                    arena = ops.ZeroArena(x.device, (len(self.convs) + 3) * (2 * ops.pad4(max(x.shape[1], conv.out_channels)) + 2))
                if sums_in is None and x.dtype == torch.float32 and x.stride(1) == 1 and x.shape[1] % 4 == 0:
                    sums_in = self._input_domain_sums(x, central_mask, arena)
                if not (conv.root_weight or conv.normalize):
                    sums = arena.take(2 * ops.pad4(conv.out_channels) + 2)
                x = conv(x, None, central_mask=central_mask, csr=csr, epilogue=(sc, sh, True), colsum=sums, sums=sums_in)
            else:
                if (ind == 0 and sums_in is None and torch.is_grad_enabled() and not x.requires_grad and x.dtype == torch.float32
                        and x.stride(1) == 1 and x.shape[1] % 4 == 0):
                    sums_in = self._input_domain_sums(x, central_mask, ops.ZeroArena(x.device, 2 * x.shape[1] + 2) if self._input_sums_miss(x, central_mask) else None)
                x = conv(x, None, central_mask=central_mask, csr=csr, sums=sums_in)
                if self.use_bn and self.training and torch.is_grad_enabled():
                    x = bn_relu_dropout_train(x, self.bns[ind], True, self.dropout)
                else:
                    if self.use_bn:
                        x = self.bns[ind](x)
                    x = F.relu(x)
                    x = F.dropout(x, p=self.dropout, training=self.training)
        self._arena = arena
        return (x, sums) if want_sums else x

    def _input_sums_miss(self, x, central_mask):
        if torch.cuda.is_current_stream_capturing() or not getattr(self, "cache_input_sums", True):
            return True
        c = getattr(self, "_xsum_cache", None)
        return not (c is not None and c[0]() is x and c[1] == x._version and c[2]() is central_mask and c[3] == central_mask._version)

    def _input_domain_sums(self, x, central_mask, arena):
        if torch.cuda.is_current_stream_capturing() or not getattr(self, "cache_input_sums", True):
            return ops.domain_sums(x, _as_u8(central_mask).contiguous(), out=arena.take(2 * x.shape[1] + 2))
        c = getattr(self, "_xsum_cache", None)
        if (c is not None and c[0]() is x and c[1] == x._version and c[2]() is central_mask and c[3] == central_mask._version):
            return c[4]
        sums = ops.domain_sums(x, _as_u8(central_mask).contiguous(), out=arena.take(2 * x.shape[1] + 2)).clone()
        self._xsum_cache = (weakref.ref(x), x._version, weakref.ref(central_mask), central_mask._version, sums)
        return sums

    def _transformer_to_target_tables(self, x, mask_u8, out, arena=None, sums_out=None):
        return self._stage.target_tables(x, mask_u8, out, arena, sums_out)

    def _composed_target_pack(self, din_pad):
        return self._stage.composed_target_pack(din_pad)

    def forward(self, data):
        x, central_mask = data.x, data.central_mask
        csr = self._prepare(data)
        x, sums_h = self._hidden(x, csr, central_mask, want_sums=True)
        x = x.contiguous()
        mask_u8 = _as_u8(central_mask).contiguous()
        stage = self._stage
        train = self.training and torch.is_grad_enabled()
        walk = stage.train_walk(opt_in=True) if (train and stage.plain and x.dtype == torch.float32) else None
        if walk is not None:
            sums_x = ops.domain_sums(_pad_cols4(x.detach()), mask_u8)
            tabs = stage.train_tables(x, mask_u8, sums_x, bn_relu_dropout_train)
            return (*stage.train_aggregate(walk, csr, mask_u8, tabs), None)
        if not stage.plain or torch.is_grad_enabled() or self.training:
            logits_base = self.clf_base(x, None, central_mask=central_mask, csr=csr)
            logits_target = self.clf_target(x, None, central_mask=central_mask, csr=csr)
            needs_grad = torch.is_grad_enabled() and (x.requires_grad or any(p.requires_grad for p in _plist(self.clf_transformer)))
            if train:
                l0, bn, _, l3 = self.clf_transformer
                xt = l3(bn_relu_dropout_train(l0(x), bn, True, 0.0))
            else:
                xt = self.clf_transformer(x) if (self.training or needs_grad) else stage.transformer_eval(x)
            logits_hat = self.clf_target(xt.contiguous(), None, central_mask=central_mask, csr=csr)
            return (F.log_softmax(logits_base, dim=1), F.log_softmax(logits_target, dim=1),
                    F.log_softmax(logits_hat, dim=1), None)
        t2s = torch.empty(x.shape[0], 3 * stage.ld, dtype=torch.float32, device=x.device)
        s2t = torch.empty_like(t2s)
        stage.eval_tables(x, mask_u8, sums_h, stage.views(t2s, s2t), self._arena)
        a_t2s, a_s2t = stage.attention()
        out3 = ops.adaptedconv_aggregate(t2s, s2t, a_t2s, a_s2t, csr, mask_u8, stage.C, stage.slope, heads=3,
                                         log_softmax=stage.fused_log_softmax)
        return (*stage.finish(out3), None)

    def graphed(self, data, warmup=2):
        if self.training:
            raise RuntimeError("graphed() captures the eval forward; call model.eval() first")
        with torch.no_grad():
            for _ in range(max(int(warmup), 1)):
                self.forward(data)
            torch.cuda.synchronize()
            g = torch.cuda.CUDAGraph()
            with torch.cuda.graph(g):
                out = self.forward(data)

        def replay():
            g.replay()
            return out
        replay.graph = g
        return replay

    def _drop_param_caches(self):
        for c in list(self.convs) + [self.clf_base, self.clf_target]:
            c._pack_key = None
        self._stage.drop_caches()
        for bn in list(self.bns) + [self.clf_transformer[1]]:
            bn._bgnn_affine = None
        _forget_plists(self)

    def invalidate_input_cache(self):
        self._xsum_cache = None

    def graphed_train_step(self, data, loss_fn, optimizer, warmup=3):
        if not self.training:
            raise RuntimeError("graphed_train_step() captures a training step; call model.train() first")
        if any(not g["capturable"] for g in optimizer.param_groups if "capturable" in g):
            raise RuntimeError("graphed_train_step() needs a capturable optimizer, e.g. torch.optim.Adam(params, capturable=True)")
        dev = data.x.device
        step = torch.zeros(1, dtype=torch.int64, device=dev)
        side = torch.cuda.Stream(device=dev)
        side.wait_stream(torch.cuda.current_stream(dev))
        _DROPOUT_STEP[0] = step
        try:
            with torch.cuda.stream(side):
                for _ in range(max(int(warmup), 1)):
                    step.add_(1)
                    optimizer.zero_grad(set_to_none=True)
                    loss_fn(self(data)).backward()
                    optimizer.step()
            torch.cuda.current_stream(dev).wait_stream(side)
            torch.cuda.synchronize(dev)
            g = torch.cuda.CUDAGraph()
            optimizer.zero_grad(set_to_none=True)
            with torch.cuda.graph(g):
                step.add_(1)
                loss = loss_fn(self(data))
                loss.backward()
                optimizer.step()
        finally:
            _DROPOUT_STEP[0] = None
        self._drop_param_caches()

        def replay():
            g.replay()
            self._drop_param_caches()
            return loss
        replay.graph, replay.step = g, step
        return replay

    def get_emb(self, data):
        return self._hidden(data.x, self._prepare(data), data.central_mask)


from . import classifier_stage
```

### bridged_gnn_amd/ops.py

```python
import ctypes
import os

import torch

from . import _lib as L

__all__ = ["DstCSR", "build_dst_csr", "domain_delta", "pack_transform_heads", "adaptedconv_transform", "adaptedconv_aggregate", "linear", "linear_supported", "linear_narrow_supported", "linear_narrow_transform", "narrow_transform_finish", "gram", "gram_supported", "rowdot", "transform_bwd_prep", "topk_edges_coalesced",
           "l2_normalize_rows", "cosine_topk", "mlp_pair_topk", "topk_edges", "coalesce", "gather_rows", "pad4",
           "sage_mean_aggregate", "sage_mean_aggregate_bwd", "rows_segment_add", "gcn_aggregate", "gcn_aggregate_bwd", "gat_scores", "gat_aggregate", "gat_aggregate_bwd", "gatv2_aggregate", "gatv2_aggregate_bwd", "wide_heads_supported",
           "adaptedconv_aggregate_heads_wide", "adaptedconv_aggregate_heads_wide_bwd", "pair_csr", "pair_mlp_stats", "pair_mlp_loss",
           "pair_mlp_segsum", "pair_mlp_eval", "pair_mlp_count", "PAIR_MLP_WIDTH", "pair_cos_loss", "pair_cos_segsum", "pair_cos_count",
           "PAIR_COS_WIDTH"]


def pad4(n):
    return (int(n) + 3) // 4 * 4


HUB_THRESHOLD = 128
HUB_SEGMENT = 64


class DstCSR:

# ... 134 lines not shown
    assert sums.numel() == 2 * Din + 2 and sums.dtype == torch.float64
    if not deterministic:
        rc = lib.bgnn_domain_sums_f64(L.ptr(x), N, Din, x.stride(0), L.ptr(mask_u8), L.ptr(sums), L.stream())
        L.check(rc, "bgnn_domain_sums_f64")
        return sums
    ws = torch.empty(lib.bgnn_domain_sums_workspace_bytes(Din), dtype=torch.uint8, device=x.device)
    rc = lib.bgnn_domain_sums_ws_f64(L.ptr(x), N, Din, x.stride(0), L.ptr(mask_u8), L.ptr(sums), L.ptr(ws), ws.numel(), L.stream())
    L.check(rc, "bgnn_domain_sums_ws_f64")
    return sums


def column_sums(x):
    N, D = x.shape
    mask = torch.zeros(N, dtype=torch.uint8, device=x.device)
    return domain_sums(x, mask)[D:2 * D].float()


def total_sum(x):
    return _TotalSumFn.apply(x)


class _TotalSumFn(torch.autograd.Function):
    @staticmethod
    def forward(ctx, x):
        ctx.shape = x.shape
        flat = x.contiguous().view(-1)
        pad = (-flat.numel()) % 64
        if pad:
            flat = torch.cat((flat, flat.new_zeros(pad)))
        return column_sums(flat.view(-1, 64)).sum()

    @staticmethod
    def backward(ctx, g):
        return g.expand(ctx.shape)


def domain_delta(sums, Din):
    delta = torch.empty(Din, dtype=torch.float32, device=sums.device)
    rc = L.lib().bgnn_domain_delta_f32(L.ptr(sums), Din, L.ptr(delta), L.stream())
    L.check(rc, "bgnn_domain_delta_f32")
    return delta


def linear_supported(din, dout):
    return din <= 128 and din % 4 == 0 and dout % 64 == 0


def linear(x, weight, bias, relu=False, mask_u8=None, colsum=None):
    N, din = x.shape
    dout = weight.shape[0]
    out = torch.empty(N, dout, dtype=torch.float32, device=x.device)
    rc = L.lib().bgnn_linear_f32(L.ptr_rows(x), N, din, x.stride(0), L.ptr(weight), L.ptr(bias), dout, 1 if relu else 0,
                                 L.ptr(mask_u8), L.ptr(colsum), L.ptr(out), dout, L.stream())
    L.check(rc, "bgnn_linear_f32")
    return out


def linear_narrow_supported(din, dout, packed):
    Wp, bp, gates, D, ldh, gconst = packed
    return (din <= 128 and din % 4 == 0 and dout in (64, 128, 256) and gates.shape[0] == 1 and ldh == 4
            and Wp.shape == (8, dout))


def linear_narrow_transform(x, weight, bias, mask_u8, colsum, packed, relu=True):
    N, din = x.shape
    dout = weight.shape[0]
    Wp, bp, gates, D, ldh, gconst = packed
    raw = torch.empty(N, 12, dtype=torch.float32, device=x.device)
    rc = L.lib().bgnn_linear_narrow_transform_f32(L.ptr_rows(x), N, din, x.stride(0), L.ptr(weight), L.ptr(bias), dout,
                                                  1 if relu else 0, L.ptr(mask_u8), L.ptr(colsum), L.ptr(Wp), L.ptr(gates),
                                                  L.ptr(raw), L.stream())
    L.check(rc, "bgnn_linear_narrow_transform_f32")
    return raw


def classifier_stage_supported(x, packed_pair, weight, packed_t):
    Wp, bp, gates, D, ldh, gconst = packed_pair
    din = x.shape[1]
    return (x.is_cuda and x.dtype == torch.float32 and x.stride(1) == 1 and 64 < din <= 128 and din % 4 == 0
            and weight.shape == (128, din) and Wp.shape[0] <= 24 and Wp.shape[1] == din and packed_t[0].shape == (8, 128)
            and os.environ.get("BGNN_FUSED_CLS", "1") != "0")


def classifier_stage(x, mask_u8, sums_x, packed_pair, outs, weight, bias, colsum, packed_t, relu=True):
    N, din = x.shape
    Wp, bp, gates, D, ldh, gconst = packed_pair
    H = gates.shape[0]
    Wp2, _, gates2, _, _, _ = packed_t
    raw = torch.empty(N, 12, dtype=torch.float32, device=x.device)
    small = torch.empty(H * (2 * ldh + 2) + 8, dtype=torch.float32, device=x.device)
    row_stride = outs[0][0].stride(0)
    for a, b in outs:
        assert a.shape[0] >= N and b.shape[0] >= N and a.stride(0) == row_stride and b.stride(0) == row_stride
    o1 = outs[1] if H > 1 else (None, None)
    rc = L.lib().bgnn_classifier_stage_f32(L.ptr_rows(x), N, din, x.stride(0), L.ptr(mask_u8), L.ptr(sums_x), H, D, L.ptr(Wp), L.ptr(bp),
                                           L.ptr(gates), L.ptr(gconst), L.ptr_rows(outs[0][1]), L.ptr_rows(outs[0][0]),
                                           L.ptr_rows(o1[1]), L.ptr_rows(o1[0]), ldh, row_stride, L.ptr(weight), L.ptr(bias),
                                           weight.shape[0], 1 if relu else 0, L.ptr(colsum), L.ptr(Wp2), L.ptr(gates2), L.ptr(raw),
                                           L.ptr(small), L.stream())
    L.check(rc, "bgnn_classifier_stage_f32")
    return raw


def narrow_transform_finish(raw, mask_u8, sums, packed, out):
    Wp, bp, gates, D, ldh, gconst = packed
    h_t2s, h_s2t = out
    N = raw.shape[0]
    assert h_t2s.stride(0) == h_s2t.stride(0) and sums.dtype == torch.float64 and sums.numel() == 2 * Wp.shape[1] + 2
    small = torch.empty(16, dtype=torch.float32, device=raw.device)
    rc = L.lib().bgnn_narrow_transform_finish_f32(L.ptr(raw), N, L.ptr(mask_u8), L.ptr(sums), Wp.shape[1], L.ptr(Wp), L.ptr(bp),
                                                  L.ptr(gates), L.ptr(gconst), L.ptr_rows(h_s2t), L.ptr_rows(h_t2s),
                                                  h_t2s.stride(0), L.ptr(small), L.stream())
    L.check(rc, "bgnn_narrow_transform_finish_f32")
    return out


def transform_bwd_prep(x, G_s2t, G_t2s, D, mask_u8, gx, gconst, wd, counts, out=None, want_ex=False):
    N, din = x.shape
    p = pad4(2 * D + 3)
    assert counts.dtype == torch.float64 and counts.numel() == 2
    if out is None:
        Gall = torch.empty(N, p, dtype=torch.float32, device=x.device)
        side = None if want_ex else torch.empty(N, 4, dtype=torch.float32, device=x.device)
    else:
        Gall, side = out
        assert Gall.shape == (N, p) and (side is None or side.shape == (N, 4))
    assert G_s2t.stride(0) == G_t2s.stride(0) and G_s2t.stride(1) == 1 and G_t2s.stride(1) == 1
    lib = L.lib()
    ex = ws = None
    wsb = 0
    if want_ex:
        ex = torch.empty(p, 4, dtype=torch.float32, device=x.device)
        wsb = lib.bgnn_transform_bwd_prep_workspace_bytes(N, p)
        ws = torch.empty(wsb, dtype=torch.uint8, device=x.device)
    rc = lib.bgnn_transform_bwd_prep_f32(L.ptr_rows(x), x.stride(0), N, din, L.ptr_rows(G_s2t), L.ptr_rows(G_t2s),
                                         G_s2t.stride(0), D, L.ptr(mask_u8), L.ptr(gx), L.ptr(gconst), L.ptr(wd),
                                         L.ptr(counts), L.ptr_rows(Gall), p, Gall.stride(0),
                                         L.ptr_rows(side) if side is not None else None, side.stride(0) if side is not None else 4,
                                         L.ptr(ex), L.ptr(ws), wsb, L.stream())
    L.check(rc, "bgnn_transform_bwd_prep_f32")
    return (Gall, ex) if want_ex else (Gall, side)


def transform_bwd_consts(W_s, W_t, g1, g2, delta, din):
    D = W_s.shape[0]
    dev = W_s.device
    gx = torch.empty(2, din, dtype=torch.float32, device=dev)
    gconst = torch.empty(2, dtype=torch.float32, device=dev)
    wd = torch.empty(2, 2 * D, dtype=torch.float32, device=dev)
    rc = L.lib().bgnn_transform_bwd_consts_f32(L.ptr(W_s), L.ptr(W_t), L.ptr(g1), L.ptr(g2), L.ptr(delta), D, din,
                                               L.ptr(gx), L.ptr(gconst), L.ptr(wd), L.stream())
    L.check(rc, "bgnn_transform_bwd_consts_f32")
    return gx, gconst, wd


def transform_bwd_finish(dWall, ex, W_s, W_t, g1, g2, delta, din, wcat_t):
    D = W_s.shape[0]
    p = dWall.shape[0]
    dev = W_s.device
    dW_s, dW_t = torch.empty(D, din, dtype=torch.float32, device=dev), torch.empty(D, din, dtype=torch.float32, device=dev)
    dg1, dg2 = torch.empty(2 * din, dtype=torch.float32, device=dev), torch.empty(2 * din, dtype=torch.float32, device=dev)
    db_s, db_t = torch.empty(D, dtype=torch.float32, device=dev), torch.empty(D, dtype=torch.float32, device=dev)
    assert dWall.is_contiguous() and ex.is_contiguous() and wcat_t.shape == (din, p) and wcat_t.stride(1) == 1
    rc = L.lib().bgnn_transform_bwd_finish_f32(L.ptr(dWall), L.ptr(ex), L.ptr(W_s), L.ptr(W_t), L.ptr(g1), L.ptr(g2), L.ptr(delta),
                                               D, din, p, L.ptr(dW_s), L.ptr(dW_t), L.ptr(dg1), L.ptr(dg2), L.ptr(db_s), L.ptr(db_t),
                                               L.ptr_rows(wcat_t), wcat_t.stride(0), L.stream())
    L.check(rc, "bgnn_transform_bwd_finish_f32")
    return dW_s, dW_t, dg1, dg2, db_s, db_t


def gram_supported(p, q):
    return 0 < p <= 288 and 0 < q <= 128 and p % 4 == 0 and q % 4 == 0


def gram(A, B):
    N, p = A.shape
    q = B.shape[1]
    lib = L.lib()
    wsb = lib.bgnn_gram_workspace_bytes(p, q)
    ws = torch.empty(wsb, dtype=torch.uint8, device=A.device)
    out = torch.empty(p, q, dtype=torch.float32, device=A.device)
    rc = lib.bgnn_gram_f32(L.ptr_rows(A), A.stride(0), p, L.ptr_rows(B), B.stride(0), q, N, L.ptr(out), L.ptr(ws), wsb, L.stream())
    L.check(rc, "bgnn_gram_f32")
    return out


def bn_relu_dropout_supported(x):
    return (x.is_cuda and x.dim() == 2 and x.dtype == torch.float32 and x.stride(1) == 1 and x.shape[1] % 4 == 0
            and 4 <= x.shape[1] <= 1024 and x.stride(0) % 4 == 0 and x.data_ptr() % 16 == 0)


def bn_relu_dropout(x, gamma, beta, eps, relu, p_drop, seed, momentum=0.0, running_mean=None, running_var=None, seed_dev=None):
    N, D = x.shape
    y = torch.empty(N, D, dtype=torch.float32, device=x.device)
    stats = torch.empty(L.lib().bgnn_bn_acc_doubles(D), dtype=torch.float64, device=x.device)
    rc = L.lib().bgnn_bn_relu_dropout_f32(L.ptr_rows(x), N, D, x.stride(0), L.ptr(gamma) if gamma is not None else None,
# ... 183 lines not shown
    runs = []
    if delta is None and H == 1 and (tile_need is not None or tail_single[0] or tail_single[1]):
        c = getattr(tile_need, "_team_plan", None)
        runs = c[1] if (c is not None and c[0] == (N, dev, tile_need._version)) else transform_team_runs(N, dev, tile_need, tail_single)
    flat = (ctypes.c_int64 * (3 * len(runs)))(*[v for r in runs for v in r]) if runs else None
    rc = lib.bgnn_adaptedconv_transform_f32(
        L.ptr(x), N, Din, x.stride(0), L.ptr(mask_u8), L.ptr(delta), None if delta is not None else L.ptr(sums), H, D, L.ptr(Wp), L.ptr(bp),
        L.ptr(gates), L.ptr(gconst), L.ptr_rows(out[0][1]), L.ptr_rows(out[0][0]), L.ptr_rows(o1[1]), L.ptr_rows(o1[0]), ldh, row_stride,
        int(tail_single[0]), int(tail_single[1]), L.ptr(tile_need), flat, len(runs), L.ptr(small), L.stream())
    L.check(rc, "bgnn_adaptedconv_transform_f32")
    return out


_P2_STATIC = os.environ.get("BGNN_P2_STATIC", "1") != "0"


_TILE_QUEUE_WORDS = None


def _tile_queue(dev):
    global _TILE_QUEUE_WORDS
    if _TILE_QUEUE_WORDS is None:
        _TILE_QUEUE_WORDS = max(8, int(L.lib().bgnn_aggregate_tile_queue_words()))
    return torch.empty(_TILE_QUEUE_WORDS, dtype=torch.int32, device=dev)


def heads_log_softmax_supported(heads, D):
    return heads in (2, 3) and D <= 4


def _hub_shape_ok(D, ldh, ldo, heads, slope):
    if heads in (2, 3) and D <= 4 and ldh == 4 and ldo == 4:
        return True
    return heads == 1 and D > 32 and 0.0 <= slope <= 1.0


def adaptedconv_aggregate(h_t2s, h_s2t, a_t2s, a_s2t, csr, mask_u8, D, negative_slope=0.1, n_dst=None,
                          want_alpha=False, ep_scale=None, ep_shift=None, ep_relu=False, out=None,
                          row_begin=0, row_end=None, state_ms=None, part=0, heads=1, colsum=None, log_softmax=False,
                          park_begin=None):
    lib = L.lib()
    n_dst = csr.num_nodes if n_dst is None else int(n_dst)
    row_end = n_dst if row_end is None else int(row_end)
    ldh = h_t2s.stride(0) // heads
    ldo = pad4(D)
    dev = h_t2s.device
    if out is None:
        out = torch.empty(n_dst, heads * ldo, dtype=torch.float32, device=dev)
    assert h_t2s.stride(0) == h_s2t.stride(0) and h_t2s.stride(0) % heads == 0 and out.stride(0) % heads == 0
    alpha = torch.empty(csr.num_edges, dtype=torch.float32, device=dev) if want_alpha else None
    tq = _tile_queue(dev) if heads == 1 else None
    if row_end <= int(row_begin):
        return (out, alpha) if want_alpha else out
    if ((not want_alpha or heads == 1) and part in (0, 3) and int(row_begin) == 0 and row_end == csr.num_nodes == n_dst and h_t2s.shape[0] == n_dst
            and (ep_scale is None or heads == 1) and _hub_shape_ok(D, ldh, out.stride(0) // heads, heads, negative_slope)
            and os.environ.get("BGNN_HUB_ROWS", "1") != "0"):
        hubs = csr.hub_tables()
        if hubs is not None:
            hub_rows, seg_ptr, seg_bounds, seg_node = hubs
            nseg = int(seg_node.numel())
            wsb = lib.bgnn_aggregate_hub_workspace_bytes(nseg, heads, out.stride(0) // heads)
            ws = torch.empty(wsb, dtype=torch.uint8, device=dev)
            rc = lib.bgnn_adaptedconv_aggregate_hub_f32(
                L.ptr_rows(h_t2s), L.ptr_rows(h_s2t), ldh, L.ptr(a_t2s), L.ptr(a_s2t), L.ptr(csr.rowptr), L.ptr(csr.col),
                L.ptr(mask_u8), n_dst, D, float(negative_slope), L.ptr_rows(out), out.stride(0) // heads,
                L.ptr(ep_scale), L.ptr(ep_shift), 2 if log_softmax else (1 if ep_relu else 0),
                L.ptr(state_ms) if part == 3 else None, int(heads), L.ptr(colsum),
                L.ptr(tq), HUB_THRESHOLD, L.ptr(hub_rows), int(hub_rows.numel()),
                L.ptr(seg_ptr), L.ptr(seg_bounds), L.ptr(seg_node), nseg, L.ptr(alpha), L.ptr(ws), wsb, L.stream())
            L.check(rc, "bgnn_adaptedconv_aggregate_hub_f32")
            return (out, alpha) if want_alpha else out
    queue = tq if not (part == 2 and _P2_STATIC) else None
    rc = lib.bgnn_adaptedconv_aggregate_queued_f32(
        L.ptr_rows(h_t2s), L.ptr_rows(h_s2t), ldh, L.ptr(a_t2s), L.ptr(a_s2t), L.ptr(csr.rowptr), L.ptr(csr.col),
        L.ptr(mask_u8), int(row_begin), row_end, D, float(negative_slope), L.ptr_rows(out), out.stride(0) // heads, L.ptr(alpha),
        L.ptr(ep_scale), L.ptr(ep_shift), 2 if log_softmax else (1 if ep_relu else 0), L.ptr(state_ms), int(part),
        int(row_begin) if park_begin is None else int(park_begin), int(heads), L.ptr(colsum),
        L.ptr(queue), 0 if queue is None else int(queue.numel()), min(int(h_t2s.shape[0]), int(h_s2t.shape[0])),
        csr.gather_hint() if (heads == 1 and D > 32 and part == 0) else 0, L.stream())
    L.check(rc, "bgnn_adaptedconv_aggregate_queued_f32")
    return (out, alpha) if want_alpha else out


def _bwd_hub_args(csr, use=True):
    use = use and os.environ.get("BGNN_HUB_ROWS", "1") != "0"
    args, nseg = [HUB_THRESHOLD], []
    for tables in ((csr.hub_tables(), csr.transposed_hub_tables()) if use else (None, None)):
        rows, seg_ptr, bounds, node = tables if tables is not None else (None, None, None, None)
        nseg.append(0 if tables is None else int(node.numel()))
        args += [L.ptr(rows), 0 if tables is None else int(rows.numel()), L.ptr(seg_ptr), L.ptr(bounds), L.ptr(node), nseg[-1]]
    return args, nseg[0], nseg[1]


def adaptedconv_aggregate_bwd(h_t2s, h_s2t, a_t2s, a_s2t, csr, mask_u8, D, out, alpha, grad_out, negative_slope=0.1):
    lib = L.lib()
    dev = h_t2s.device
    da_t2s = torch.zeros(D, dtype=torch.float32, device=dev)
    da_s2t = torch.zeros(D, dtype=torch.float32, device=dev)
    grad_out = grad_out.contiguous()
    ldh, ldo, ldg = h_t2s.stride(0), out.stride(0), grad_out.stride(0)
    pull = D <= 256 and ldg % 4 == 0 and grad_out.data_ptr() % 16 == 0 and h_t2s.shape[0] == csr.num_nodes
    if pull and D > 128:
        pull = (ldh % 4 == 0 and ldo % 4 == 0 and h_t2s.data_ptr() % 16 == 0 and h_s2t.data_ptr() % 16 == 0
                and out.data_ptr() % 16 == 0)
    if pull:
        t_rowptr, t_eid, t_dst = csr.transposed()
        dh_t2s, dh_s2t = torch.empty_like(h_t2s), torch.empty_like(h_s2t)
        narrow = D <= 4 and ldh == 4 and ldo == 4 and ldg == 4
        hub_args, nd, ns = _bwd_hub_args(csr, use=not narrow)
        wsb = lib.bgnn_aggregate_bwd_pull_workspace_bytes(csr.num_nodes, csr.num_edges, ldh, D, nd, ns)
        ws = torch.empty(wsb, dtype=torch.uint8, device=dev)
        rc = lib.bgnn_adaptedconv_aggregate_bwd_pull_f32(
            L.ptr(h_t2s), L.ptr(h_s2t), ldh, L.ptr(a_t2s), L.ptr(a_s2t), L.ptr(csr.rowptr), L.ptr(csr.col),
            L.ptr(mask_u8), L.ptr(t_rowptr), L.ptr(t_eid), L.ptr(t_dst), csr.num_nodes, csr.num_edges, D, float(negative_slope),
            L.ptr(out), ldo, L.ptr(alpha), L.ptr(grad_out), ldg,
            L.ptr(dh_t2s), L.ptr(dh_s2t), L.ptr(da_t2s), L.ptr(da_s2t), *hub_args, L.ptr(ws), wsb, L.stream())
        L.check(rc, "bgnn_adaptedconv_aggregate_bwd_pull_f32")
        return dh_t2s, dh_s2t, da_t2s, da_s2t
    dh_t2s, dh_s2t = torch.zeros_like(h_t2s), torch.zeros_like(h_s2t)
    rc = lib.bgnn_adaptedconv_aggregate_bwd_f32(
        L.ptr(h_t2s), L.ptr(h_s2t), ldh, L.ptr(a_t2s), L.ptr(a_s2t), L.ptr(csr.rowptr), L.ptr(csr.col),
        L.ptr(mask_u8), 0, csr.num_nodes, D, float(negative_slope), L.ptr(out), ldo, L.ptr(alpha),
        L.ptr(grad_out), ldg, L.ptr(dh_t2s), L.ptr(dh_s2t), L.ptr(da_t2s), L.ptr(da_s2t), L.stream())
    L.check(rc, "bgnn_adaptedconv_aggregate_bwd_f32")
    return dh_t2s, dh_s2t, da_t2s, da_s2t


def adaptedconv_aggregate_heads_bwd(t2s, s2t, a_t2s, a_s2t, csr, mask_u8, D, heads, out, state_ms, grad_out, log_softmax,
                                    negative_slope=0.1):
    lib = L.lib()
    dev = t2s.device
    N = csr.num_nodes
    assert t2s.shape == (N, heads * 4) and t2s.is_contiguous() and s2t.is_contiguous() and out.is_contiguous() and grad_out.is_contiguous()
    da_t2s = torch.zeros(heads, D, dtype=torch.float32, device=dev)
    da_s2t = torch.zeros(heads, D, dtype=torch.float32, device=dev)
    dh_t2s, dh_s2t = torch.empty_like(t2s), torch.empty_like(s2t)
    t_rowptr, _, t_dst = csr.transposed()
    hub_args, nd, ns = _bwd_hub_args(csr)
    wsb = lib.bgnn_aggregate_heads_bwd_workspace_bytes(N, csr.num_edges, heads, nd, ns)
    ws = torch.empty(wsb, dtype=torch.uint8, device=dev)
    rc = lib.bgnn_adaptedconv_aggregate_heads_bwd_f32(
        L.ptr(t2s), L.ptr(s2t), L.ptr(a_t2s), L.ptr(a_s2t), L.ptr(csr.rowptr), L.ptr(csr.col), L.ptr(mask_u8),
        L.ptr(t_rowptr), L.ptr(t_dst), N, csr.num_edges, D, heads, float(negative_slope),
        L.ptr(out), L.ptr(state_ms), L.ptr(grad_out), int(bool(log_softmax)), L.ptr(dh_t2s), L.ptr(dh_s2t),
        L.ptr(da_t2s), L.ptr(da_s2t), *hub_args, L.ptr(ws), wsb, L.stream())
    L.check(rc, "bgnn_adaptedconv_aggregate_heads_bwd_f32")
    return dh_t2s, dh_s2t, da_t2s, da_s2t


def wide_heads_supported(heads, D):
    return heads in (2, 3) and 4 < int(D) <= 32


def adaptedconv_aggregate_heads_wide(t2s, s2t, a_t2s, a_s2t, csr, mask_u8, D, heads, negative_slope=0.1):
    lib = L.lib()
    N, ld = csr.num_nodes, pad4(D)
    assert t2s.shape == (N, heads * ld) and s2t.shape == t2s.shape and t2s.is_contiguous() and s2t.is_contiguous()
    out = torch.empty(N, heads * ld, dtype=torch.float32, device=t2s.device)
    ms = torch.empty(N, heads, 2, dtype=torch.float32, device=t2s.device)
    rc = lib.bgnn_adaptedconv_aggregate_heads_wide_f32(
        L.ptr(t2s), L.ptr(s2t), ld, L.ptr(a_t2s), L.ptr(a_s2t), L.ptr(csr.rowptr), L.ptr(csr.col), L.ptr(mask_u8),
        N, int(D), int(heads), float(negative_slope), L.ptr(out), L.ptr(ms), L.stream())
    L.check(rc, "bgnn_adaptedconv_aggregate_heads_wide_f32")
    return out, ms


# ... 1172 lines not shown
```

### include/bgnn.h

```cpp
#ifndef BGNN_H_
#define BGNN_H_
#include <stddef.h>
#include <stdint.h>

#ifdef __cplusplus
extern "C" {
#endif

#define BGNN_VERSION 116
#define BGNN_E_NULL (-1)
#define BGNN_E_SHAPE (-2)
#define BGNN_E_WORKSPACE (-3)
#define BGNN_E_ALIGN (-4)
#define BGNN_E_RANGE (-5)

int bgnn_version(void);
const char* bgnn_error_string(int code);
const char* bgnn_source_hash(void);

size_t bgnn_csr_workspace_bytes(int64_t N, int64_t E);
int bgnn_build_dst_csr(const int64_t* edge_index, int64_t E, int64_t N, int rewrite_self_loops,
                       int32_t* rowptr, int32_t* col, int32_t* eperm_opt, int64_t* E_out_dev,
                       void* ws, size_t ws_bytes, void* stream);

int bgnn_domain_sums_f64(const float* x, int64_t N, int32_t Din, int64_t ldx, const uint8_t* mask,
                         double* sums_io , void* stream);
size_t bgnn_domain_sums_workspace_bytes(int32_t Din);
int bgnn_domain_sums_ws_f64(const float* x, int64_t N, int32_t Din, int64_t ldx, const uint8_t* mask,
                            double* sums_io , void* ws, size_t ws_bytes, void* stream);
int bgnn_domain_delta_f32(const double* sums , int32_t Din, float* delta, void* stream);
int bgnn_linear_f32(const float* x, int64_t N, int32_t Din, int64_t ldx, const float* W, const float* bias,
                    int32_t Dout, int relu, const uint8_t* mask_opt, double* colsum_opt,
                    float* out, int64_t ldo, void* stream);
int bgnn_linear_narrow_transform_f32(const float* x, int64_t N, int32_t Din, int64_t ldx, const float* W,
                                     const float* bias, int32_t Dout, int relu, const uint8_t* mask,
                                     double* colsum, const float* Wp2, const float* gates2, float* raw, void* stream);
int bgnn_classifier_stage_f32(const float* x, int64_t N, int32_t Din, int64_t ldx, const uint8_t* mask,
                              const double* sums_x, int32_t sk_heads, int32_t sk_D, const float* sk_Wp,
                              const float* sk_bias, const float* sk_gates, const float* sk_gate_const_opt,
                              float* h_s2t_0, float* h_t2s_0, float* h_s2t_1, float* h_t2s_1, int64_t sk_ldh,
                              int64_t sk_row_stride, const float* W, const float* bias, int32_t Dout, int relu,
                              double* colsum, const float* Wp2, const float* gates2, float* raw, float* small_ws,
                              void* stream);
int bgnn_narrow_transform_finish_f32(const float* raw, int64_t N, const uint8_t* mask, const double* sums,
                                     int32_t Din, const float* Wp2, const float* bias2, const float* gates2,
                                     const float* gate_const_opt, float* h_s2t, float* h_t2s, int64_t row_stride,
                                     float* small_ws, void* stream);
size_t bgnn_gram_workspace_bytes(int32_t p, int32_t q);
int bgnn_gram_f32(const float* A, int64_t lda, int32_t p, const float* B, int64_t ldb, int32_t q, int64_t N,
                  float* out , void* ws, size_t ws_bytes, void* stream);
int64_t bgnn_bn_acc_doubles(int32_t D);
int bgnn_bn_relu_dropout_f32(const float* x, int64_t N, int32_t D, int64_t ldx, const float* gamma_opt,
                             const float* beta_opt, float eps, int relu, float p_drop, uint64_t seed, const uint64_t* seed_dev_opt,
                             float momentum, float* running_mean_opt, float* running_var_opt,
                             float* y, int64_t ldy, double* stats, void* stream);
int bgnn_bn_relu_dropout_bwd_f32(const float* x, const float* grad_y, int64_t N, int32_t D, int64_t ldx, int64_t ldg,
                                 const double* stats, const float* gamma_opt, const float* beta_opt, float eps,
                                 int relu, float p_drop, uint64_t seed, const uint64_t* seed_dev_opt, float* grad_x, int64_t ldgx,
                                 double* gsum, void* stream);
int bgnn_bn_colstats_f32(const float* x, int64_t n_rows, int32_t D, int64_t ldx, double* acc, void* stream);
int bgnn_bn_apply_rows_f32(const float* x, int64_t n_rows, int32_t D, int64_t ldx, const double* totals, int64_t n_total,
                           const float* gamma_opt, const float* beta_opt, float eps, int relu, float p_drop, uint64_t seed,
                           const uint64_t* seed_dev_opt, const int64_t* row_ids_opt, int64_t row_base,
                           float momentum, float* running_mean_opt, float* running_var_opt,
                           float* y, int64_t ldy, void* stream);
int bgnn_bn_bwd_reduce_rows_f32(const float* x, const float* grad_y, int64_t n_rows, int32_t D, int64_t ldx, int64_t ldg,
                                const double* totals, int64_t n_total, const float* gamma_opt, const float* beta_opt,
                                float eps, int relu, float p_drop, uint64_t seed, const uint64_t* seed_dev_opt,
                                const int64_t* row_ids_opt, int64_t row_base, double* gacc, void* stream);
int bgnn_bn_bwd_apply_rows_f32(const float* x, const float* grad_y, int64_t n_rows, int32_t D, int64_t ldx, int64_t ldg,
                               const double* totals, const double* gtotals, int64_t n_total, const float* gamma_opt,
                               const float* beta_opt, float eps, int relu, float p_drop, uint64_t seed,
                               const uint64_t* seed_dev_opt, const int64_t* row_ids_opt, int64_t row_base,
                               float* grad_x, int64_t ldgx, void* stream);
size_t bgnn_transform_bwd_prep_workspace_bytes(int64_t N, int32_t p);
int bgnn_transform_bwd_prep_f32(const float* x, int64_t ldx, int64_t N, int32_t din, const float* G_s2t, const float* G_t2s,
                                int64_t ldg, int32_t D, const uint8_t* mask, const float* gx ,
                                const float* gconst , const float* wd , const double* counts ,
                                float* Gall, int32_t p, int64_t ld_gall, float* side_opt, int64_t ld_side,
                                float* ex_opt , void* ws_opt, size_t ws_bytes, void* stream);
int bgnn_transform_bwd_consts_f32(const float* W_s, const float* W_t, const float* g1, const float* g2, const float* delta,
                                  int32_t D, int32_t din, float* gx, float* gconst, float* wd, void* stream);
int bgnn_transform_bwd_finish_f32(const float* dWall, const float* ex, const float* W_s, const float* W_t, const float* g1,
                                  const float* g2, const float* delta, int32_t D, int32_t din, int32_t p, float* dW_s,
                                  float* dW_t, float* dg1, float* dg2, float* db_s_opt, float* db_t_opt, float* wcat_t,
                                  int64_t ld_wcat, void* stream);
int bgnn_rowdot_f32(const float* X, int64_t ldx, int64_t N, int32_t d, const float* V, int64_t ldv, int32_t nv,
                    float* out , void* stream);
int bgnn_adaptedconv_transform_f32(const float* x, int64_t N, int32_t Din, int64_t ldx,
                                   const uint8_t* mask, const float* delta_opt, const double* sums_opt,
                                   int32_t n_heads, int32_t D, const float* Wp, const float* bias_p,
                                   const float* gates, const float* gate_const_opt,
                                   float* h_s2t_0, float* h_t2s_0, float* h_s2t_1, float* h_t2s_1,
                                   int64_t ldh, int64_t row_stride, int64_t n_tail_t2s, int64_t n_tail_s2t,
                                   const int32_t* tile_need_opt, const int64_t* team_runs_host_opt, int32_t n_team_runs,
                                   float* small_ws, void* stream);

int bgnn_adaptedconv_aggregate_f32(const float* h_t2s, const float* h_s2t, int64_t ldh,
                                   const float* a_t2s, const float* a_s2t,
                                   const int32_t* rowptr, const int32_t* col, const uint8_t* mask,
                                   int64_t row_begin, int64_t row_end, int32_t D, float negative_slope,
                                   float* out, int64_t ldo, float* alpha_opt,
                                   const float* ep_scale_opt, const float* ep_shift_opt, int ep_relu,
                                   float* state_ms_opt, int part, int64_t park_begin, int32_t heads, double* colsum_opt,
                                   uint32_t* tile_queue_opt, void* stream);

int bgnn_adaptedconv_aggregate_bounded_f32(const float* h_t2s, const float* h_s2t, int64_t ldh,
                                           const float* a_t2s, const float* a_s2t,
                                           const int32_t* rowptr, const int32_t* col, const uint8_t* mask,
                                           int64_t row_begin, int64_t row_end, int32_t D, float negative_slope,
                                           float* out, int64_t ldo, float* alpha_opt,
                                           const float* ep_scale_opt, const float* ep_shift_opt, int ep_relu,
                                           float* state_ms_opt, int part, int64_t park_begin, int32_t heads, double* colsum_opt,
                                           uint32_t* tile_queue_opt, int64_t table_rows, int32_t gather_hint, void* stream);

int64_t bgnn_aggregate_tile_queue_words(void);
int bgnn_adaptedconv_aggregate_queued_f32(const float* h_t2s, const float* h_s2t, int64_t ldh,
                                          const float* a_t2s, const float* a_s2t,
                                          const int32_t* rowptr, const int32_t* col, const uint8_t* mask,
                                          int64_t row_begin, int64_t row_end, int32_t D, float negative_slope,
                                          float* out, int64_t ldo, float* alpha_opt,
                                          const float* ep_scale_opt, const float* ep_shift_opt, int ep_relu,
                                          float* state_ms_opt, int part, int64_t park_begin, int32_t heads, double* colsum_opt,
                                          uint32_t* tile_queue_opt, int64_t tile_queue_words, int64_t table_rows, int32_t gather_hint,
                                          void* stream);

size_t bgnn_aggregate_hub_workspace_bytes(int64_t n_segments, int32_t heads, int64_t ldo);
int bgnn_adaptedconv_aggregate_hub_f32(const float* h_t2s, const float* h_s2t, int64_t ldh,
                                       const float* a_t2s, const float* a_s2t,
                                       const int32_t* rowptr, const int32_t* col, const uint8_t* mask,
// ... 272 lines not shown
```

Baseline: 53.45 billion edges/s.

## Pack classifier head tables into 32-byte rows for eval aggregation

Adds a compact table layout for the 3-head, C<=2 eval classifier path: each node's three heads are packed into 8 floats (2+2+4) per direction instead of 12. The producer kernels write this layout directly, and a new aggregation kernel gathers one 32-byte row per neighbour with buffer loads and a two-lanes-per-edge split. The aim is to cut the bytes fetched per edge in the gather-bound edge aggregation. It brings in a new specialised kernel with hand-written inline-asm pipelining, and it falls back to the old path whenever hub tables exist or the shape checks fail.

```diff
diff --git a/bridged_gnn_amd/_lib.py b/bridged_gnn_amd/_lib.py
--- a/bridged_gnn_amd/_lib.py
+++ b/bridged_gnn_amd/_lib.py
@@ -25,6 +25,11 @@
                                           _P, _P, _I32, _INT, _P, _P, _P, _P, _P, _P]),
     "bgnn_linear_narrow_transform_f32": (_INT, [_P, _I64, _I32, _I64, _P, _P, _I32, _INT, _P, _P, _P, _P, _P, _P]),
     "bgnn_narrow_transform_finish_f32": (_INT, [_P, _I64, _P, _P, _I32, _P, _P, _P, _P, _P, _P, _I64, _P, _P]),
+    "bgnn_classifier_stage_rows32_f32": (_INT, [_P, _I64, _I32, _I64, _P, _P, _I32, _P, _P, _P, _P, _P, _P, _I64,
+                                                 _P, _P, _I32, _INT, _P, _P, _P, _P, _P, _P]),
+    "bgnn_narrow_transform_finish_rows32_f32": (_INT, [_P, _I64, _P, _P, _I32, _P, _P, _P, _P, _P, _P, _I64, _P, _P]),
+    "bgnn_adaptedconv_aggregate_heads_rows32_plan": (_INT, [_P, _P, _I64, _I64, _I32, _F32]),
+    "bgnn_adaptedconv_aggregate_heads_rows32_f32": (_INT, [_P, _P, _P, _P, _P, _P, _P, _I64, _I64, _I32, _F32, _P, _INT, _I64, _P]),
     "bgnn_gram_workspace_bytes": (C.c_size_t, [_I32, _I32]),
     "bgnn_gram_f32": (_INT, [_P, _I64, _I32, _P, _I64, _I32, _I64, _P, _P, C.c_size_t, _P]),
     "bgnn_transform_bwd_prep_workspace_bytes": (C.c_size_t, [_I64, _I32]),
diff --git a/bridged_gnn_amd/classifier_stage.py b/bridged_gnn_amd/classifier_stage.py
--- a/bridged_gnn_amd/classifier_stage.py
+++ b/bridged_gnn_amd/classifier_stage.py
@@ -23,6 +23,38 @@
     def views(self, t2s, s2t):
         ld = self.ld
         return [(t2s[:, j * ld:(j + 1) * ld], s2t[:, j * ld:(j + 1) * ld]) for j in range(3)]
+
+    def rows32_eligible(self, dtype=torch.float32, training=False):
+        return self.plain and self.C <= 2 and dtype == torch.float32 and not training
+
+    @staticmethod
+    def rows32_views(t2s, s2t):
+        return [(t2s[:, 0:2], s2t[:, 0:2]), (t2s[:, 2:4], s2t[:, 2:4]), (t2s[:, 4:8], s2t[:, 4:8])]
+
+    @staticmethod
+    def rows32_pack(tab):
+        t = tab.view(tab.shape[0], 3, 4)
+        return torch.cat((t[:, 0, :2], t[:, 1, :2], t[:, 2, :]), dim=1).contiguous()
+
+    @staticmethod
+    def rows32_unpack(tab8):
+        out = tab8.new_zeros(tab8.shape[0], 3, 4)
+        out[:, 0, :2], out[:, 1, :2], out[:, 2, :] = tab8[:, 0:2], tab8[:, 2:4], tab8[:, 4:8]
+        return out.view(tab8.shape[0], 12)
+
+    def eval_tables_rows32(self, x, mask_u8, sums_h, csr, arena):
+        if not self.rows32_eligible(x.dtype) or x.stride(1) != 1:
+            return None
+        ops_a = self._one_pass_operands(x, sums_h)
+        if ops_a is None:
+            return None
+        both = torch.empty(2, x.shape[0], 8, dtype=torch.float32, device=x.device)
+        t2s, s2t = both[0], both[1]
+        if not ops.heads_rows32_plan(t2s, s2t, csr, self.C, self.slope, row_end=x.shape[0]):
+            return None
+        a = self.one_pass(x, mask_u8, sums_h, None, arena, rows32=(t2s, s2t), operands=ops_a)
+        self.target_stage_b(a, mask_u8, self.rows32_views(t2s, s2t)[2], rows32=True)
+        return t2s, s2t
 
     def attention(self, autograd=False):
         if autograd:
@@ -91,7 +123,7 @@
             self._tf_pack = (key, ops.pack_transform_heads([head], din_pad))
         return self._tf_pack[1]
 
-    def one_pass(self, x, mask_u8, sums_h, views, arena):
+    def _one_pass_operands(self, x, sums_h):
         if sums_h is None or x.dtype != torch.float32 or x.stride(1) != 1:
             return None
         self.fold_transformer()
@@ -102,9 +134,18 @@
         pair = self.convs[0].packed(x.shape[1], self.convs[1])
         if not ops.classifier_stage_supported(x, pair, self._tf_w0, pack_t):
             return None
-        n_s = 2 * ops.pad4(dout) + 2
+        return pair, pack_t
+
+    def one_pass(self, x, mask_u8, sums_h, views, arena, rows32=None, operands=None):
+        if operands is None:
+            operands = self._one_pass_operands(x, sums_h)
+        if operands is None:
+            return None
+        pair, pack_t = operands
+        n_s = 2 * ops.pad4(self._tf_w0.shape[0]) + 2
         sums_t = arena.take(n_s) if arena is not None else torch.zeros(n_s, dtype=torch.float64, device=x.device)
-        raw = ops.classifier_stage(x, mask_u8, sums_h, pair, [views[0], views[1]], self._tf_w0, self._tf_b0, sums_t, pack_t, relu=True)
+        outs = [views[0], views[1]] if rows32 is None else None
+        raw = ops.classifier_stage(x, mask_u8, sums_h, pair, outs, self._tf_w0, self._tf_b0, sums_t, pack_t, relu=True, rows32=rows32)
         return raw, None, sums_t
 
     def pair_tables(self, x, mask_u8, sums_h, views):
@@ -123,11 +164,12 @@
             sums1 = ops.domain_sums(h1, mask_u8)
         return None, h1, sums1
 
-    def target_stage_b(self, stage_a, mask_u8, out, sums_t=None):
+    def target_stage_b(self, stage_a, mask_u8, out, sums_t=None, rows32=False):
         raw, h1, sums_t = (*stage_a[:2], sums_t if sums_t is not None else stage_a[2])
         if raw is not None:
-            ops.narrow_transform_finish(raw, mask_u8, sums_t, self.composed_target_pack(ops.pad4(self._tf_w0.shape[0])), out)
+            ops.narrow_transform_finish(raw, mask_u8, sums_t, self.composed_target_pack(ops.pad4(self._tf_w0.shape[0])), out, rows32=rows32)
         else:
+            assert not rows32
             ops.adaptedconv_transform(h1, mask_u8, None, self.composed_target_pack(h1.shape[1]), out=[out], sums=sums_t)
 
     def target_tables(self, x, mask_u8, out, arena=None, sums_out=None):
diff --git a/bridged_gnn_amd/csrc/bgnn_aggregate.hip b/bridged_gnn_amd/csrc/bgnn_aggregate.hip
--- a/bridged_gnn_amd/csrc/bgnn_aggregate.hip
+++ b/bridged_gnn_amd/csrc/bgnn_aggregate.hip
@@ -1156,6 +1156,187 @@
   }
 }
 
+__global__ __launch_bounds__(256) __attribute__((amdgpu_waves_per_eu(BGNN_HEADS_FAST_WAVES))) void agg_heads_rows32_kernel(AggParams p) {
+  constexpr int EP = 2, U = 4, GPW = 16, RPB = 4 * GPW;
+  constexpr uint32_t RS = 32u;
+  constexpr int32_t STEP = EP * U;
+  const int lane = threadIdx.x & 63, wave = threadIdx.x >> 6;
+  const int g = lane >> 2, sub = (lane >> 1) & 1, part = lane & 1;
+  const int32_t row0 = (int32_t)p.row_begin, row1 = (int32_t)p.row_end;
+  const int32_t ntiles = (row1 - row0 + RPB - 1) / RPB;
+  const uint64_t tb = (uint64_t)p.tbl_base;
+  const u32x4_t rt = {(uint32_t)tb, (uint32_t)(tb >> 32) & 0xffffu, p.tbl_bytes, 0x00020000u};
+  const __amdgpu_buffer_rsrc_t rtb = __builtin_amdgcn_make_buffer_rsrc(const_cast<char*>(p.tbl_base), (short)0, (int)p.tbl_bytes, 0x00020000);
+  const __amdgpu_buffer_rsrc_t ro = __builtin_amdgcn_make_buffer_rsrc(p.out, (short)0, (int)((uint32_t)row1 * 48u), 0x00020000);
+  const uint32_t dead = p.dead_off;
+  const uint32_t cend = (uint32_t)p.rowptr[row1] * 4u;
+  const int pidx = (lane ^ 2) * 4;
+  const f2 sl = {p.slope, p.slope};
+  __shared__ float4 a_lds[2][2];
+  if (threadIdx.x < 4) {
+    const float* a = threadIdx.x < 2 ? p.a_s2t : p.a_t2s;
+    const int h0 = (threadIdx.x & 1) * 2;
+    float4 v;
+    v.x = a[h0 * p.D];
+    v.y = p.D > 1 ? a[h0 * p.D + 1] : 0.f;
+    v.z = h0 == 0 ? a[p.D] : 0.f;
+    v.w = (h0 == 0 && p.D > 1) ? a[p.D + 1] : 0.f;
+    a_lds[threadIdx.x >> 1][threadIdx.x & 1] = v;
+  }
+  __syncthreads();
+  const int32_t per = (ntiles + 7) / 8, seg_len = (per + bgnn::XCD_NSEG - 1) / bgnn::XCD_NSEG;
+  const int32_t xcd = blockIdx.x % 8, nslots = ((int32_t)gridDim.x + 7 - xcd) / 8;
+  int32_t sg = 0, r = blockIdx.x / 8;
+  for (;; r += nslots) {
+    while (r >= seg_len) { r -= seg_len; ++sg; }
+    if (sg >= bgnn::XCD_NSEG) break;
+    const int32_t tile = (sg * 8 + xcd) * seg_len + r;
+    if (tile >= ntiles) continue;
+    const int32_t i = row0 + tile * RPB + wave * GPW + g;
+    const bool rvalid = i < row1;
+    const int32_t ic = rvalid ? i : row0;
+    const bool dom_s = p.mask[ic] != 0;
+    const int32_t rp0 = p.rowptr[ic], rp1 = p.rowptr[ic + 1];
+    const int32_t beg = rvalid ? rp0 : 0, end = rvalid ? rp1 : 0;
+    const uint32_t lbase = (dom_s ? p.off_t2s : p.off_s2t) + (uint32_t)part * 16u;
+    const float4 a4 = a_lds[dom_s ? 1 : 0][part];
+    f4v_t hi = __builtin_bit_cast(f4v_t, __builtin_amdgcn_raw_buffer_load_b128(rtb, lbase + __umul24((uint32_t)ic, RS), 0, 0));
+    f2 accA = {0.f, 0.f}, accB = {0.f, 0.f};
+    float mA = -INFINITY, sA = 0.f, mB = -INFINITY, sB = 0.f;
+    const int32_t niter = (int32_t)((uint32_t)(end - beg + STEP - 1) / (uint32_t)STEP);
+    int32_t rem = end - beg - sub;
+    const int32_t bfirst = __builtin_amdgcn_readfirstlane(beg);
+    const bool slow = __builtin_amdgcn_ballot_w64(rvalid && (uint32_t)(end + (end - bfirst) + 16) * 4u > cend) != 0;
+    const uint32_t elast = (uint32_t)max(end - 1, 0) * 4u;
+    uint32_t off[U] = {dead, dead, dead, dead};
+    const bool any = __builtin_amdgcn_ballot_w64(niter > 0) != 0;
+    auto walk = [&](auto slow_tag) {
+      constexpr bool SLOW = decltype(slow_tag)::value;
+      uint32_t xoff = SLOW ? (uint32_t)(beg + sub) * 4u : (uint32_t)((rvalid ? beg : bfirst) + 4 * sub) * 4u;
+      auto request = [&](u32x4_t& q) {
+        __builtin_amdgcn_sched_barrier(0);
+        if constexpr (SLOW) {
+          uint32_t eo[U];
+#pragma unroll
+          for (int u = 0; u < U; ++u) eo[u] = min(xoff + (uint32_t)(u * EP * 4), elast);
+          asm volatile("global_load_dword %0, %1, %2" : "=v"(q.x) : "v"(eo[0]), "s"(p.col) : "memory");
+          asm volatile("global_load_dword %0, %1, %2" : "=v"(q.y) : "v"(eo[1]), "s"(p.col) : "memory");
+          asm volatile("global_load_dword %0, %1, %2" : "=v"(q.z) : "v"(eo[2]), "s"(p.col) : "memory");
+          asm volatile("global_load_dword %0, %1, %2" : "=v"(q.w) : "v"(eo[3]), "s"(p.col) : "memory");
+        } else {
+          asm volatile("global_load_dwordx4 %0, %1, %2" : "=v"(q) : "v"(xoff), "s"(p.col) : "memory");
+        }
+        __builtin_amdgcn_sched_barrier(0);
+      };
+      auto take = [&](u32x4_t& q, uint32_t (&id)[U]) {
+        __builtin_amdgcn_sched_barrier(0);
+        asm volatile("s_waitcnt vmcnt(0)" : "+v"(q), "+v"(mA), "+v"(sA), "+v"(accA), "+v"(mB), "+v"(sB), "+v"(accB) : : "memory");
+        if constexpr (SLOW) {
+          id[0] = q.x; id[1] = q.y; id[2] = q.z; id[3] = q.w;
+        } else {
+          const uint32_t r0 = (uint32_t)__builtin_amdgcn_ds_bpermute(pidx, (int)(sub ? q.x : q.y));
+          const uint32_t r1 = (uint32_t)__builtin_amdgcn_ds_bpermute(pidx, (int)(sub ? q.z : q.w));
+          id[0] = sub ? r0 : q.x; id[1] = sub ? r1 : q.z; id[2] = sub ? q.y : r0; id[3] = sub ? q.w : r1;
+        }
+        __builtin_amdgcn_sched_barrier(0);
+      };
+      auto offsets = [&](const uint32_t (&id)[U]) {
+#pragma unroll
+        for (int u = 0; u < U; ++u) off[u] = rem > u * EP ? lbase + __umul24(id[u], RS) : dead;
+      };
+      {
+        uint32_t id[U];
+        u32x4_t q;
+        request(q);
+        take(q, id);
+        offsets(id);
+      }
+      asm volatile("" : "+v"(hi) : : "memory");
+      const f2 hA = {hi.x, hi.y}, hB = {hi.z, hi.w};
+      for (int32_t it = 0; __builtin_amdgcn_ballot_w64(it < niter) != 0; ++it) {
+        f4v_t v[U];
+        __builtin_amdgcn_sched_barrier(0);
+#pragma unroll
+        for (int u = 0; u < U; ++u) asm volatile("buffer_load_dwordx4 %0, %1, %2, 0 offen" : "=v"(v[u]) : "v"(off[u]), "s"(rt) : "memory");
+        xoff += (uint32_t)(STEP * 4);
+        u32x4_t nq;
+        request(nq);
+        if constexpr (SLOW) asm volatile("s_waitcnt vmcnt(4)" : "+v"(v[0]), "+v"(v[1]), "+v"(v[2]), "+v"(v[3]) : : "memory");
+        else asm volatile("s_waitcnt vmcnt(1)" : "+v"(v[0]), "+v"(v[1]), "+v"(v[2]), "+v"(v[3]) : : "memory");
+        __builtin_amdgcn_sched_barrier(0);
+        float lA[U], lB[U], cmA = -INFINITY, cmB = -INFINITY;
+#pragma unroll
+        for (int u = 0; u < U; ++u) {
+          f2 zA = f2{v[u].x, v[u].y} + hA, zB = f2{v[u].z, v[u].w} + hB;
+          zA = __builtin_elementwise_max(zA, zA * sl);
+          zB = __builtin_elementwise_max(zB, zB * sl);
+          float tA = a4.x * zA.x;
+          tA = fmaf(a4.y, zA.y, tA);
+          float tB = a4.z * zB.x;
+          tB = fmaf(a4.w, zB.y, tB);
+          lA[u] = rem > u * EP ? tA : -INFINITY;
+          lB[u] = rem > u * EP ? tB : -INFINITY;
+          cmA = fmaxf(cmA, lA[u]);
+          cmB = fmaxf(cmB, lB[u]);
+        }
+        const float mnA = fmaxf(mA, cmA), mnB = fmaxf(mB, cmB);
+        const float scA = (mA == mnA) ? 1.f : __expf(mA - mnA), scB = (mB == mnB) ? 1.f : __expf(mB - mnB);
+        accA *= f2{scA, scA}; accB *= f2{scB, scB};
+#pragma unroll
+        for (int u = 0; u < U; ++u) {
+          const float peA = (lA[u] == -INFINITY) ? 0.f : __expf(lA[u] - mnA);
+          const float peB = (lB[u] == -INFINITY) ? 0.f : __expf(lB[u] - mnB);
+          sA = u == 0 ? fmaf(sA, scA, peA) : sA + peA;
+          sB = u == 0 ? fmaf(sB, scB, peB) : sB + peB;
+          accA.x = fmaf(peA, v[u].x, accA.x); accA.y = fmaf(peA, v[u].y, accA.y);
+          accB.x = fmaf(peB, v[u].z, accB.x); accB.y = fmaf(peB, v[u].w, accB.y);
+        }
+        mA = mnA; mB = mnB;
+        rem -= STEP;
+        uint32_t nid[U];
+        take(nq, nid);
+        offsets(nid);
+      }
+    };
+    if (any) {
+      if (slow) walk(std::true_type{});
+      else walk(std::false_type{});
+    }
+    {
+      const int from = lane ^ 2;
+      const float mA2 = __shfl(mA, from), sA2 = __shfl(sA, from), mB2 = __shfl(mB, from), sB2 = __shfl(sB, from);
+      f2 bA, bB;
+      bA.x = __shfl(accA.x, from); bA.y = __shfl(accA.y, from); bB.x = __shfl(accB.x, from); bB.y = __shfl(accB.y, from);
+      const float mnA = fmaxf(mA, mA2), mnB = fmaxf(mB, mB2);
+      const float cA1 = (mA == mnA) ? 1.f : __expf(mA - mnA), cA2 = (mA2 == mnA) ? 1.f : __expf(mA2 - mnA);
+      const float cB1 = (mB == mnB) ? 1.f : __expf(mB - mnB), cB2 = (mB2 == mnB) ? 1.f : __expf(mB2 - mnB);
+      sA = fmaf(sA, cA1, sA2 * cA2); sB = fmaf(sB, cB1, sB2 * cB2);
+      accA.x = fmaf(accA.x, cA1, bA.x * cA2); accA.y = fmaf(accA.y, cA1, bA.y * cA2);
+      accB.x = fmaf(accB.x, cB1, bB.x * cB2); accB.y = fmaf(accB.y, cB1, bB.y * cB2);
+    }
+    if (rvalid && sub == 0) {
+#pragma clang fp contract(off)
+      auto finish = [&](float s, f2 acc) {
+        const float inv = 1.f / (s + 1e-16f);
+        float4 r4 = make_float4(acc.x * inv, acc.y * inv, 0.f, 0.f);
+        if (p.ep_relu == 2) {
+          float mx = r4.x;
+          if (p.D > 1) mx = fmaxf(mx, r4.y);
+          float se = expf(r4.x - mx);
+          if (p.D > 1) se += expf(r4.y - mx);
+          const float lse = logf(se);
+          r4.x = r4.x - mx - lse;
+          r4.y = p.D > 1 ? r4.y - mx - lse : 0.f;
+        }
+        return __builtin_bit_cast(u32x4_t, r4);
+      };
+      const uint32_t o = ((uint32_t)i * 3u + (uint32_t)part * 2u) * 16u;
+      __builtin_amdgcn_raw_buffer_store_b128(finish(sA, accA), ro, o, 0, 0);
+      if (part == 0) __builtin_amdgcn_raw_buffer_store_b128(finish(sB, accB), ro, o + 16u, 0, 0);
+    }
+  }
+}
+
 inline int tq_chunk_for(int64_t ntiles, int64_t grid) {
   static const int forced = [] { const char* e = getenv("BGNN_AGG_CHUNK"); return e ? atoi(e) : 0; }();
   (void)ntiles; (void)grid;
@@ -1256,14 +1437,17 @@
   return true;
 }
 
-static bool heads_fast_plan(AggParams& p, int64_t table_rows) {
+constexpr bool kHeadsRows32Default = true;
+static bool heads_fast_plan(AggParams& p, int64_t table_rows, bool rows32 = false) {
   static const bool on = [] { const char* e = getenv("BGNN_HEADS_FAST"); return !(e && atoi(e) == 0); }();
   if (!on || table_rows <= 0) return false;
   if ((p.heads != 2 && p.heads != 3) || p.D > 4 || p.ldh != 4 || p.ldo != 4) return false;
   if (p.mode != 0 || p.n_vrows != 0 || p.hub_threshold != 0 || p.alpha != nullptr) return false;
   if (!(p.slope >= 0.f && p.slope <= 1.f)) return false;
   const int64_t lim24 = (int64_t)1 << 24, lim32 = ((int64_t)1 << 32) - 1;
-  const int64_t rs = (int64_t)p.heads * 16;
+  static const bool on32 = [] { const char* e = getenv("BGNN_HEADS_ROWS32"); return e ? atoi(e) != 0 : kHeadsRows32Default; }();
+  if (rows32 && (!on32 || p.heads != 3 || p.D > 2)) return false;
+  const int64_t rs = rows32 ? 32 : (int64_t)p.heads * 16;
   if (table_rows > lim24 || p.row_end > table_rows) return false;
   const char* a = reinterpret_cast<const char*>(p.h_t2s);
   const char* b = reinterpret_cast<const char*>(p.h_s2t);
@@ -1482,6 +1666,24 @@
   return 0;
 }
 
+static int launch_heads_rows32(const AggParams& p, hipStream_t st) {
+  constexpr int RPB = 64;
+  static const int cap = [] {
+    int per_cu = 0, dev = 0;
+    hipDeviceProp_t prop;
+    if (hipGetDevice(&dev) != hipSuccess || hipGetDeviceProperties(&prop, dev) != hipSuccess) return 2048;
+    if (hipOccupancyMaxActiveBlocksPerMultiprocessor(&per_cu, agg_heads_rows32_kernel, 256, 0) != hipSuccess || per_cu < 1) return 2048;
+    if (per_cu > 8) per_cu = 8;
+    return per_cu * prop.multiProcessorCount / 8 * 8;
+  }();
+  const int64_t ntiles = (p.row_end - p.row_begin + RPB - 1) / RPB;
+  int64_t grid = ntiles < cap ? (ntiles + 7) / 8 * 8 : cap;
+  if (grid < 8) grid = 8;
+  hipLaunchKernelGGL(agg_heads_rows32_kernel, dim3((unsigned)grid), dim3(256), 0, st, p);
+  BGNN_LAUNCH_CHECK();
+  return 0;
+}
+
 static int dispatch_aggregate(const AggParams& p, hipStream_t st, int64_t table_rows = 0) {
   const int32_t D = p.D, heads = p.heads;
   if ((heads == 3 || heads == 2) && D <= 4 && p.ldh == 4 && p.ldo == 4) {
@@ -1585,6 +1787,35 @@
   if (table_rows < row_end || gather_hint < 0 || gather_hint > 2) return BGNN_E_SHAPE;
   return aggregate_impl(h_t2s, h_s2t, ldh, a_t2s, a_s2t, rowptr, col, mask, row_begin, row_end, D, negative_slope, out, ldo, alpha_opt,
                         ep_scale_opt, ep_shift_opt, ep_relu, state_ms_opt, part, park_begin, heads, colsum_opt, tile_queue_opt, 8, table_rows, gather_hint, stream);
+}
+
+static int rows32_params(AggParams& p, const float* t_t2s, const float* t_s2t, const float* a_t2s, const float* a_s2t,
+                         const int32_t* rowptr, const int32_t* col, const uint8_t* mask, int64_t row_begin, int64_t row_end,
+                         int32_t D, float negative_slope, float* out, int ep_relu, int64_t table_rows) {
+  if (!t_t2s || !t_s2t) return BGNN_E_NULL;
+  if (row_begin < 0 || row_end < row_begin || table_rows < row_end || D <= 0 || D > 2 || (ep_relu != 0 && ep_relu != 2)) return BGNN_E_SHAPE;
+  if (!bgnn_aligned16(t_t2s) || !bgnn_aligned16(t_s2t) || (out && !bgnn_aligned16(out))) return BGNN_E_ALIGN;
+  p = AggParams{t_t2s, t_s2t, 4, a_t2s, a_s2t, rowptr, col, mask, row_begin, row_end, D, negative_slope,
+                out, 4, nullptr, nullptr, nullptr, ep_relu, nullptr, nullptr, 3, nullptr, 0, row_begin, 4};
+  return heads_fast_plan(p, table_rows, true) ? 0 : BGNN_E_SHAPE;
+}
+
+extern "C" int bgnn_adaptedconv_aggregate_heads_rows32_plan(const float* t_t2s, const float* t_s2t, int64_t table_rows,
+                                                            int64_t row_end, int32_t D, float negative_slope) {
+  AggParams p;
+  return rows32_params(p, t_t2s, t_s2t, nullptr, nullptr, nullptr, nullptr, nullptr, 0, row_end, D, negative_slope, nullptr, 0, table_rows) == 0;
+}
+
+extern "C" int bgnn_adaptedconv_aggregate_heads_rows32_f32(const float* t_t2s, const float* t_s2t, const float* a_t2s, const float* a_s2t,
+                                                           const int32_t* rowptr, const int32_t* col, const uint8_t* mask,
+                                                           int64_t row_begin, int64_t row_end, int32_t D, float negative_slope,
+                                                           float* out, int ep_relu, int64_t table_rows, void* stream) {
+  if (!a_t2s || !a_s2t || !rowptr || !col || !mask || !out) return BGNN_E_NULL;
+  AggParams p;
+  const int rc = rows32_params(p, t_t2s, t_s2t, a_t2s, a_s2t, rowptr, col, mask, row_begin, row_end, D, negative_slope, out, ep_relu, table_rows);
+  if (rc) return rc;
+  if (row_end == row_begin) return 0;
+  return launch_heads_rows32(p, (hipStream_t)stream);
 }
 
 extern "C" int64_t bgnn_aggregate_tile_queue_words(void) { return claim_cfg().tile ? claim_queue_words() : 8; }
diff --git a/bridged_gnn_amd/csrc/bgnn_transform.hip b/bridged_gnn_amd/csrc/bgnn_transform.hip
--- a/bridged_gnn_amd/csrc/bgnn_transform.hip
+++ b/bridged_gnn_amd/csrc/bgnn_transform.hip
@@ -940,7 +940,7 @@
                                                             const uint8_t* __restrict__ mask,
                                                             const float* __restrict__ bias, const float* __restrict__ wd,
                                                             const float* __restrict__ gc, float* __restrict__ out_s2t,
-                                                            float* __restrict__ out_t2s, int64_t row_stride) {
+                                                            float* __restrict__ out_t2s, int64_t row_stride, int rows32) {
   const float4 b0 = *reinterpret_cast<const float4*>(bias), b1 = *reinterpret_cast<const float4*>(bias + 4);
   const float4 w0 = *reinterpret_cast<const float4*>(wd), w1 = *reinterpret_cast<const float4*>(wd + 4);
   const float g0 = gc[0], g1 = gc[1];
@@ -956,6 +956,7 @@
     o0.z = fmaf(c0, w0.z, a.z + b0.z); o0.w = fmaf(c0, w0.w, a.w + b0.w);
     o1.x = fmaf(c1, w1.x, b.x + b1.x); o1.y = fmaf(c1, w1.y, b.y + b1.y);
     o1.z = fmaf(c1, w1.z, b.z + b1.z); o1.w = fmaf(c1, w1.w, b.w + b1.w);
+    if (rows32) o0.z = o0.w = o1.z = o1.w = 0.f;
     *reinterpret_cast<float4*>(out_s2t + r * row_stride) = o0;
     *reinterpret_cast<float4*>(out_t2s + r * row_stride) = o1;
   }
@@ -978,13 +979,13 @@
   return launch_wreg<2>(p, (hipStream_t)stream);
 }
 
-extern "C" int bgnn_classifier_stage_f32(const float* x, int64_t N, int32_t Din, int64_t ldx, const uint8_t* mask,
-                                         const double* sums_x, int32_t sk_heads, int32_t sk_D, const float* sk_Wp,
-                                         const float* sk_bias, const float* sk_gates, const float* sk_gate_const_opt,
-                                         float* h_s2t_0, float* h_t2s_0, float* h_s2t_1, float* h_t2s_1, int64_t sk_ldh,
-                                         int64_t sk_row_stride, const float* W, const float* bias, int32_t Dout, int relu,
-                                         double* colsum, const float* Wp2, const float* gates2, float* raw, float* small_ws,
-                                         void* stream) {
+static int classifier_stage_impl(const float* x, int64_t N, int32_t Din, int64_t ldx, const uint8_t* mask,
+                                 const double* sums_x, int32_t sk_heads, int32_t sk_D, const float* sk_Wp,
+                                 const float* sk_bias, const float* sk_gates, const float* sk_gate_const_opt,
+                                 float* h_s2t_0, float* h_t2s_0, float* h_s2t_1, float* h_t2s_1, int64_t sk_ldh,
+                                 int64_t sk_row_stride, const float* W, const float* bias, int32_t Dout, int relu,
+                                 double* colsum, const float* Wp2, const float* gates2, float* raw, float* small_ws,
+                                 void* stream, int rows32) {
   if (!x || !mask || !sums_x || !sk_Wp || !sk_bias || !sk_gates || !h_s2t_0 || !h_t2s_0 || !W || !bias || !colsum || !Wp2 || !gates2 ||
       !raw || !small_ws) return BGNN_E_NULL;
   if (sk_heads < 1 || sk_heads > MAXH || (sk_heads == 2 && (!h_s2t_1 || !h_t2s_1))) return BGNN_E_NULL;
@@ -1003,7 +1004,7 @@
   p.w2 = Wp2; p.g2 = gates2; p.raw = raw;
   p.sk_Wp = sk_Wp; p.sk_bias = sk_bias; p.sk_wd = wd; p.sk_g = sk_gates; p.sk_gc = gc;
   p.sk_out[0][0] = h_s2t_0; p.sk_out[0][1] = h_t2s_0; p.sk_out[1][0] = h_s2t_1; p.sk_out[1][1] = h_t2s_1;
-  p.sk_ldh = sk_ldh; p.sk_row_stride = sk_row_stride; p.sk_NC = sk_NC; p.sk_heads = sk_heads;
+  p.sk_ldh = sk_ldh; p.sk_row_stride = sk_row_stride; p.sk_NC = sk_NC; p.sk_heads = sk_heads; p.sk_rows32 = rows32;
   if (!bgnn_tf_cls_supported(p)) return BGNN_E_SHAPE;
   hipLaunchKernelGGL(wd_kernel, dim3((unsigned)((sk_NC + 2 * sk_heads + 3) / 4)), dim3(256), 0, st, sk_Wp, sk_NC, Din, (const float*)nullptr,
                      sums_x, sk_gates, sk_gate_const_opt, sk_heads, wd, gc);
@@ -1011,10 +1012,33 @@
   return bgnn_tf_cls_launch(p, st, n_cu());
 }
 
-extern "C" int bgnn_narrow_transform_finish_f32(const float* raw, int64_t N, const uint8_t* mask, const double* sums,
-                                                int32_t Din, const float* Wp2, const float* bias2, const float* gates2,
-                                                const float* gate_const_opt, float* h_s2t, float* h_t2s,
-                                                int64_t row_stride, float* small_ws, void* stream) {
+extern "C" int bgnn_classifier_stage_f32(const float* x, int64_t N, int32_t Din, int64_t ldx, const uint8_t* mask,
+                                         const double* sums_x, int32_t sk_heads, int32_t sk_D, const float* sk_Wp,
+                                         const float* sk_bias, const float* sk_gates, const float* sk_gate_const_opt,
+                                         float* h_s2t_0, float* h_t2s_0, float* h_s2t_1, float* h_t2s_1, int64_t sk_ldh,
+                                         int64_t sk_row_stride, const float* W, const float* bias, int32_t Dout, int relu,
+                                         double* colsum, const float* Wp2, const float* gates2, float* raw, float* small_ws,
+                                         void* stream) {
+  return classifier_stage_impl(x, N, Din, ldx, mask, sums_x, sk_heads, sk_D, sk_Wp, sk_bias, sk_gates, sk_gate_const_opt, h_s2t_0, h_t2s_0,
+                               h_s2t_1, h_t2s_1, sk_ldh, sk_row_stride, W, bias, Dout, relu, colsum, Wp2, gates2, raw, small_ws, stream, 0);
+}
+
+extern "C" int bgnn_classifier_stage_rows32_f32(const float* x, int64_t N, int32_t Din, int64_t ldx, const uint8_t* mask,
+                                                const double* sums_x, int32_t sk_D, const float* sk_Wp, const float* sk_bias,
+                                                const float* sk_gates, const float* sk_gate_const_opt, float* t_s2t, float* t_t2s,
+                                                int64_t sk_row_stride, const float* W, const float* bias, int32_t Dout, int relu,
+                                                double* colsum, const float* Wp2, const float* gates2, float* raw, float* small_ws,
+                                                void* stream) {
+  if (sk_D > 2) return BGNN_E_SHAPE;
+  if (!bgnn_aligned16(t_s2t) || !bgnn_aligned16(t_t2s)) return BGNN_E_ALIGN;
+  return classifier_stage_impl(x, N, Din, ldx, mask, sums_x, 2, sk_D, sk_Wp, sk_bias, sk_gates, sk_gate_const_opt, t_s2t, t_t2s, t_s2t, t_t2s,
+                               4, sk_row_stride, W, bias, Dout, relu, colsum, Wp2, gates2, raw, small_ws, stream, 1);
+}
+
+static int narrow_finish_impl(const float* raw, int64_t N, const uint8_t* mask, const double* sums,
+                              int32_t Din, const float* Wp2, const float* bias2, const float* gates2,
+                              const float* gate_const_opt, float* h_s2t, float* h_t2s,
+                              int64_t row_stride, float* small_ws, void* stream, int rows32) {
   if (!raw || !mask || !sums || !Wp2 || !bias2 || !gates2 || !h_s2t || !h_t2s || !small_ws) return BGNN_E_NULL;
   if (N < 0 || Din <= 0 || (Din & 3) || row_stride < 4 || (row_stride & 3)) return BGNN_E_SHAPE;
   if (!bgnn_aligned16(raw) || !bgnn_aligned16(h_s2t) || !bgnn_aligned16(h_t2s) || !bgnn_aligned16(bias2) ||
@@ -1027,7 +1051,21 @@
   BGNN_LAUNCH_CHECK();
   const int64_t nb = (N + 255) / 256;
   hipLaunchKernelGGL(narrow_finish_kernel, dim3((unsigned)(nb < 4096 ? nb : 4096)), dim3(256), 0, st, raw, N, mask, bias2, wd, gc,
-                     h_s2t, h_t2s, row_stride);
+                     h_s2t, h_t2s, row_stride, rows32);
   BGNN_LAUNCH_CHECK();
   return 0;
 }
+
+extern "C" int bgnn_narrow_transform_finish_f32(const float* raw, int64_t N, const uint8_t* mask, const double* sums,
+                                                int32_t Din, const float* Wp2, const float* bias2, const float* gates2,
+                                                const float* gate_const_opt, float* h_s2t, float* h_t2s,
+                                                int64_t row_stride, float* small_ws, void* stream) {
+  return narrow_finish_impl(raw, N, mask, sums, Din, Wp2, bias2, gates2, gate_const_opt, h_s2t, h_t2s, row_stride, small_ws, stream, 0);
+}
+
+extern "C" int bgnn_narrow_transform_finish_rows32_f32(const float* raw, int64_t N, const uint8_t* mask, const double* sums,
+                                                       int32_t Din, const float* Wp2, const float* bias2, const float* gates2,
+                                                       const float* gate_const_opt, float* h_s2t, float* h_t2s,
+                                                       int64_t row_stride, float* small_ws, void* stream) {
+  return narrow_finish_impl(raw, N, mask, sums, Din, Wp2, bias2, gates2, gate_const_opt, h_s2t, h_t2s, row_stride, small_ws, stream, 1);
+}
diff --git a/bridged_gnn_amd/csrc/bgnn_transform_cls.hip b/bridged_gnn_amd/csrc/bgnn_transform_cls.hip
--- a/bridged_gnn_amd/csrc/bgnn_transform_cls.hip
+++ b/bridged_gnn_amd/csrc/bgnn_transform_cls.hip
@@ -265,7 +265,7 @@
       CLS_MARK(2);
       const float ss = s_row * cinvS;
       if (valid) {
-        float cf = 0.f;
+        float cf = 0.f, k0 = 0.f, k1 = 0.f;
 #pragma unroll
         for (int q = 0; q < 3; ++q) {
           if (optr[q] != nullptr) {
@@ -278,7 +278,9 @@
             float4 o;
             o.x = fmaf(cf, wq.x, fmaf(acc[4 * q], ss, bq.x));     o.y = fmaf(cf, wq.y, fmaf(acc[4 * q + 1], ss, bq.y));
             o.z = fmaf(cf, wq.z, fmaf(acc[4 * q + 2], ss, bq.z)); o.w = fmaf(cf, wq.w, fmaf(acc[4 * q + 3], ss, bq.w));
-            *reinterpret_cast<float4*>(optr[q] + row * p.sk_row_stride) = o;
+            if (!p.sk_rows32) *reinterpret_cast<float4*>(optr[q] + row * p.sk_row_stride) = o;
+            else if (q == 0) { k0 = o.x; k1 = o.y; }
+            else *reinterpret_cast<float4*>(optr[0] + row * p.sk_row_stride) = make_float4(k0, k1, o.x, o.y);
           }
         }
       }
diff --git a/bridged_gnn_amd/csrc/bgnn_transform_params.h b/bridged_gnn_amd/csrc/bgnn_transform_params.h
--- a/bridged_gnn_amd/csrc/bgnn_transform_params.h
+++ b/bridged_gnn_amd/csrc/bgnn_transform_params.h
@@ -28,6 +28,7 @@
   int32_t team_table[2];
   const float* sk_Wp; const float* sk_bias; const float* sk_wd; const float* sk_g; const float* sk_gc;
   float* sk_out[MAXH][2]; int64_t sk_ldh; int64_t sk_row_stride; int32_t sk_NC; int32_t sk_heads;
+  int32_t sk_rows32;
 };
 
 __device__ __forceinline__ float tanh_fast(float z) { return 1.f - 2.f * __builtin_amdgcn_rcpf(__expf(2.f * z) + 1.f); }
diff --git a/bridged_gnn_amd/ktgnn.py b/bridged_gnn_amd/ktgnn.py
--- a/bridged_gnn_amd/ktgnn.py
+++ b/bridged_gnn_amd/ktgnn.py
@@ -716,10 +716,15 @@
             logits_hat = self.clf_target(xt.contiguous(), None, central_mask=central_mask, csr=csr)
             return (F.log_softmax(logits_base, dim=1), F.log_softmax(logits_target, dim=1),
                     F.log_softmax(logits_hat, dim=1), None)
+        a_t2s, a_s2t = stage.attention()
+        tabs = stage.eval_tables_rows32(x, mask_u8, sums_h, csr, self._arena)
+        if tabs is not None:
+            out3 = ops.adaptedconv_aggregate_heads_rows32(*tabs, a_t2s, a_s2t, csr, mask_u8, stage.C, stage.slope,
+                                                          log_softmax=stage.fused_log_softmax)
+            return (*stage.finish(out3), None)
         t2s = torch.empty(x.shape[0], 3 * stage.ld, dtype=torch.float32, device=x.device)
         s2t = torch.empty_like(t2s)
         stage.eval_tables(x, mask_u8, sums_h, stage.views(t2s, s2t), self._arena)
-        a_t2s, a_s2t = stage.attention()
         out3 = ops.adaptedconv_aggregate(t2s, s2t, a_t2s, a_s2t, csr, mask_u8, stage.C, stage.slope, heads=3,
                                          log_softmax=stage.fused_log_softmax)
         return (*stage.finish(out3), None)
diff --git a/bridged_gnn_amd/ops.py b/bridged_gnn_amd/ops.py
--- a/bridged_gnn_amd/ops.py
+++ b/bridged_gnn_amd/ops.py
@@ -240,13 +240,22 @@
             and os.environ.get("BGNN_FUSED_CLS", "1") != "0")
 
 
-def classifier_stage(x, mask_u8, sums_x, packed_pair, outs, weight, bias, colsum, packed_t, relu=True):
+def classifier_stage(x, mask_u8, sums_x, packed_pair, outs, weight, bias, colsum, packed_t, relu=True, rows32=None):
     N, din = x.shape
     Wp, bp, gates, D, ldh, gconst = packed_pair
     H = gates.shape[0]
     Wp2, _, gates2, _, _, _ = packed_t
     raw = torch.empty(N, 12, dtype=torch.float32, device=x.device)
     small = torch.empty(H * (2 * ldh + 2) + 8, dtype=torch.float32, device=x.device)
+    if rows32 is not None:
+        t2s, s2t = rows32
+        assert H == 2 and ldh == 4 and D <= 2 and t2s.shape[0] >= N and s2t.shape[0] >= N and t2s.stride(0) == s2t.stride(0)
+        rc = L.lib().bgnn_classifier_stage_rows32_f32(L.ptr_rows(x), N, din, x.stride(0), L.ptr(mask_u8), L.ptr(sums_x), D, L.ptr(Wp),
+                                                      L.ptr(bp), L.ptr(gates), L.ptr(gconst), L.ptr_rows(s2t), L.ptr_rows(t2s),
+                                                      t2s.stride(0), L.ptr(weight), L.ptr(bias), weight.shape[0], 1 if relu else 0,
+                                                      L.ptr(colsum), L.ptr(Wp2), L.ptr(gates2), L.ptr(raw), L.ptr(small), L.stream())
+        L.check(rc, "bgnn_classifier_stage_rows32_f32")
+        return raw
     row_stride = outs[0][0].stride(0)
     for a, b in outs:
         assert a.shape[0] >= N and b.shape[0] >= N and a.stride(0) == row_stride and b.stride(0) == row_stride
@@ -260,16 +269,18 @@
     return raw
 
 
-def narrow_transform_finish(raw, mask_u8, sums, packed, out):
+def narrow_transform_finish(raw, mask_u8, sums, packed, out, rows32=False):
     Wp, bp, gates, D, ldh, gconst = packed
     h_t2s, h_s2t = out
     N = raw.shape[0]
     assert h_t2s.stride(0) == h_s2t.stride(0) and sums.dtype == torch.float64 and sums.numel() == 2 * Wp.shape[1] + 2
+    assert not rows32 or D <= 2
     small = torch.empty(16, dtype=torch.float32, device=raw.device)
-    rc = L.lib().bgnn_narrow_transform_finish_f32(L.ptr(raw), N, L.ptr(mask_u8), L.ptr(sums), Wp.shape[1], L.ptr(Wp), L.ptr(bp),
-                                                  L.ptr(gates), L.ptr(gconst), L.ptr_rows(h_s2t), L.ptr_rows(h_t2s),
-                                                  h_t2s.stride(0), L.ptr(small), L.stream())
-    L.check(rc, "bgnn_narrow_transform_finish_f32")
+    name = "bgnn_narrow_transform_finish_rows32_f32" if rows32 else "bgnn_narrow_transform_finish_f32"
+    rc = getattr(L.lib(), name)(L.ptr(raw), N, L.ptr(mask_u8), L.ptr(sums), Wp.shape[1], L.ptr(Wp), L.ptr(bp),
+                                L.ptr(gates), L.ptr(gconst), L.ptr_rows(h_s2t), L.ptr_rows(h_t2s),
+                                h_t2s.stride(0), L.ptr(small), L.stream())
+    L.check(rc, name)
     return out
 
 
@@ -619,6 +630,30 @@
     return (out, alpha) if want_alpha else out
 
 
+def heads_rows32_plan(t2s, s2t, csr, D, negative_slope, row_end=None):
+    if not (t2s.is_cuda and t2s.dtype == s2t.dtype == torch.float32 and t2s.dim() == s2t.dim() == 2 and t2s.shape[1] == s2t.shape[1] == 8
+            and t2s.stride() == s2t.stride() == (8, 1)):
+        return False
+    if os.environ.get("BGNN_HUB_ROWS", "1") != "0" and csr.hub_tables() is not None:
+        return False
+    rows = min(int(t2s.shape[0]), int(s2t.shape[0]))
+    row_end = csr.num_nodes if row_end is None else int(row_end)
+    return bool(L.lib().bgnn_adaptedconv_aggregate_heads_rows32_plan(L.ptr(t2s), L.ptr(s2t), rows, row_end, int(D), float(negative_slope)))
+
+
+def adaptedconv_aggregate_heads_rows32(t2s, s2t, a_t2s, a_s2t, csr, mask_u8, D, negative_slope=0.1, log_softmax=False,
+                                       row_begin=0, row_end=None, out=None):
+    row_end = csr.num_nodes if row_end is None else int(row_end)
+    if out is None:
+        out = torch.empty(csr.num_nodes, 12, dtype=torch.float32, device=t2s.device)
+    assert t2s.stride() == s2t.stride() == (8, 1) and out.stride() == (12, 1) and out.shape[0] >= row_end
+    rc = L.lib().bgnn_adaptedconv_aggregate_heads_rows32_f32(
+        L.ptr(t2s), L.ptr(s2t), L.ptr(a_t2s), L.ptr(a_s2t), L.ptr(csr.rowptr), L.ptr(csr.col), L.ptr(mask_u8), int(row_begin), row_end,
+        int(D), float(negative_slope), L.ptr(out), 2 if log_softmax else 0, min(int(t2s.shape[0]), int(s2t.shape[0])), L.stream())
+    L.check(rc, "bgnn_adaptedconv_aggregate_heads_rows32_f32")
+    return out
+
+
 def _bwd_hub_args(csr, use=True):
     use = use and os.environ.get("BGNN_HUB_ROWS", "1") != "0"
     args, nseg = [HUB_THRESHOLD], []
diff --git a/include/bgnn.h b/include/bgnn.h
--- a/include/bgnn.h
+++ b/include/bgnn.h
@@ -46,6 +46,22 @@
                                      int32_t Din, const float* Wp2, const float* bias2, const float* gates2,
                                      const float* gate_const_opt, float* h_s2t, float* h_t2s, int64_t row_stride,
                                      float* small_ws, void* stream);
+int bgnn_classifier_stage_rows32_f32(const float* x, int64_t N, int32_t Din, int64_t ldx, const uint8_t* mask,
+                                     const double* sums_x, int32_t sk_D, const float* sk_Wp, const float* sk_bias,
+                                     const float* sk_gates, const float* sk_gate_const_opt, float* t_s2t, float* t_t2s,
+                                     int64_t sk_row_stride, const float* W, const float* bias, int32_t Dout, int relu,
+                                     double* colsum, const float* Wp2, const float* gates2, float* raw, float* small_ws,
+                                     void* stream);
+int bgnn_narrow_transform_finish_rows32_f32(const float* raw, int64_t N, const uint8_t* mask, const double* sums,
+                                            int32_t Din, const float* Wp2, const float* bias2, const float* gates2,
+                                            const float* gate_const_opt, float* h_s2t, float* h_t2s, int64_t row_stride,
+                                            float* small_ws, void* stream);
+int bgnn_adaptedconv_aggregate_heads_rows32_plan(const float* t_t2s, const float* t_s2t, int64_t table_rows, int64_t row_end,
+                                                 int32_t D, float negative_slope);
+int bgnn_adaptedconv_aggregate_heads_rows32_f32(const float* t_t2s, const float* t_s2t, const float* a_t2s, const float* a_s2t,
+                                                const int32_t* rowptr, const int32_t* col, const uint8_t* mask,
+                                                int64_t row_begin, int64_t row_end, int32_t D, float negative_slope,
+                                                float* out, int ep_relu, int64_t table_rows, void* stream);
 size_t bgnn_gram_workspace_bytes(int32_t p, int32_t q);
 int bgnn_gram_f32(const float* A, int64_t lda, int32_t p, const float* B, int64_t ldb, int32_t q, int64_t N,
                   float* out , void* ws, size_t ws_bytes, void* stream);
```

New measurement: 55.29 billion edges/s (median of 6 runs). +3.4%, better.
